# nalinbhardwaj/curdleproofs.pie

Hardware: AMD Instinct MI355X
Metric: BLS12-381 G1 scalar-muls/sec at MSM size 2^20 (higher is better)
Workload: dtype u32

## Files before the change

curdleproofs_pie_amd/csrc/capi_core_msm.h:

```cpp
#pragma once

using cg1::Ctx;
struct cg1_ctx : public cg1::Ctx {};

namespace cg1 {
static Ctx* child_of(Ctx* ctx) { return static_cast<Ctx*>(ctx->child); }

static int ensure_child(Ctx* ctx) {
  if (!ctx->child) {
    cg1_ctx* made = ctx->cu_mask.empty() ? cg1_ctx_create(ctx->device) : cg1_ctx_create_cu_mask(ctx->device, ctx->cu_mask.data(), ctx->cu_mask.size());
    if (!made) { snprintf(ctx->err, sizeof ctx->err, "could not create the second launch chain's context"); return CG1_ERR_HIP; }
    made->split = 0;
    made->batched_split = 0;
    ctx->child = made;
  }
  if (!ctx->ev_prep) HIPCHK(hipEventCreateWithFlags(&ctx->ev_prep, hipEventDisableTiming));
  if (!ctx->ev_acc) HIPCHK(hipEventCreateWithFlags(&ctx->ev_acc, hipEventDisableTiming));
  return CG1_OK;
}

static int msm_begin_split(Ctx* ctx, const PtSrc& src, const void* d_scalars32, size_t n, const WinPlan& plan, int rank, int world) {
  HIPCHK(hipSetDevice(ctx->device));
  { int crc = ensure_child(ctx); if (crc) return crc; }
  Ctx* ch = child_of(ctx);
  ch->profile = ctx->profile; ch->L0 = ctx->L0; ch->seg_m = ctx->seg_m; ch->quad = ctx->quad; ch->reduce_2d = ctx->reduce_2d;
  ch->rowcol_quad = ctx->rowcol_quad; ch->rowcol_quad_max = ctx->rowcol_quad_max; ch->fold_pass = ctx->fold_pass; ch->tree_half = ctx->tree_half; ch->tree_shift = ctx->tree_shift; ch->rowcol_lgq = ctx->rowcol_lgq; ch->tree_row = ctx->tree_row; ch->rowcol_row = ctx->rowcol_row; ch->sort_sub_bits = ctx->sort_sub_bits;
  ch->scan_one = ctx->scan_one; ch->zero_copy = ctx->zero_copy; ch->horner_threads = ctx->horner_threads; ch->host_split = ctx->host_split;
  ch->blocking_sync = ctx->blocking_sync; ch->stage_sort = ctx->stage_sort; ch->use_partition_sort = ctx->use_partition_sort; ch->big_bins = ctx->big_bins;
  const int n_own = win_count(plan.nwin, rank, world), n_lo = n_own / 2, n_hi = n_own - n_lo;
  ChainHooks hi;
  hi.after_prepare = ctx->ev_prep; hi.after_accumulate = ctx->ev_acc;
  int rc = msm_enqueue(ctx, src, d_scalars32, n, plan, rank, win_sel(world, n_lo, n_hi), hi);
  if (rc) return rc;
  PtSrc shared;
  shared.kind = PtSrc::PREPARED;
  shared.p = src.kind == PtSrc::PREPARED ? src.p : ctx->d_pts;
  shared.flags = src.kind == PtSrc::PREPARED ? src.flags : ctx->d_flags;
  ChainHooks lo;
  lo.before_start = ctx->ev_prep; lo.before_accumulate = ctx->ev_acc;
  rc = msm_enqueue(ch, shared, d_scalars32, n, plan, rank, win_sel(world, 0, n_lo), lo);
  if (rc) { snprintf(ctx->err, sizeof ctx->err, "%s", ch->err); cg1h::jac dummy; (void)msm_finish(ctx, dummy); return rc; }
  ctx->pend_split = true;
  return CG1_OK;
}
}

namespace {
struct DevBuf {
  void* p = nullptr;
  ~DevBuf() { if (p) (void)hipFree(p); }
  hipError_t alloc(size_t bytes) { return hipMalloc(&p, bytes ? bytes : 16); }
};
}

static inline cg1h::jac blob_in(const uint8_t* b) { cg1h::jac j; memcpy(&j, b, sizeof j); return j; }
static inline void blob_out(uint8_t* b, const cg1h::jac& j) { memcpy(b, &j, sizeof j); }
static_assert(sizeof(cg1h::jac) == CG1_POINT_BYTES, "point blob size");

extern "C" {

void cg1_identity(uint8_t* out) { blob_out(out, cg1h::jac_identity()); }
void cg1_generator(uint8_t* out) { blob_out(out, cg1h::jac_generator()); }
void cg1_add(uint8_t* out, const uint8_t* a, const uint8_t* b) { blob_out(out, cg1h::jac_add(blob_in(a), blob_in(b))); }
void cg1_sub(uint8_t* out, const uint8_t* a, const uint8_t* b) { blob_out(out, cg1h::jac_add(blob_in(a), cg1h::jac_neg(blob_in(b)))); }
void cg1_neg(uint8_t* out, const uint8_t* a) { blob_out(out, cg1h::jac_neg(blob_in(a))); }
void cg1_double(uint8_t* out, const uint8_t* a) { blob_out(out, cg1h::jac_dbl(blob_in(a))); }
void cg1_mul(uint8_t* out, const uint8_t* a, const uint8_t* k) { blob_out(out, cg1h::jac_mul(blob_in(a), k)); }
int cg1_eq(const uint8_t* a, const uint8_t* b) { return cg1h::jac_eq(blob_in(a), blob_in(b)) ? 1 : 0; }
int cg1_is_identity(const uint8_t* a) { return cg1h::jac_is_identity(blob_in(a)) ? 1 : 0; }
void cg1_compress(uint8_t* out48, const uint8_t* a) { cg1h::g1_compress(blob_in(a), out48); }
static int map_dec(int rc) {
  switch (rc) { case 0: return CG1_OK; case 1: case 2: return CG1_ERR_ENCODING; case 3: return CG1_ERR_NOT_ON_CURVE; default: return CG1_ERR_NOT_IN_SUBGROUP; }
}
int cg1_decompress(uint8_t* out, const uint8_t* in48, int check_subgroup) {
  cg1h::jac j;
  int rc = cg1h::g1_decompress(in48, check_subgroup != 0, j);
  if (rc == 0) blob_out(out, j);
  return map_dec(rc);
}
void cg1_to_affine96(uint8_t* out96, const uint8_t* a) {
  cg1h::fe x, y; bool inf;
  cg1h::jac_to_affine(blob_in(a), x, y, inf);
  if (inf) { memset(out96, 0, 96); return; }
  cg1h::fe_to_le48(x, out96); cg1h::fe_to_le48(y, out96 + 48);
}
int cg1_from_affine96(uint8_t* out, const uint8_t* in96, int check_on_curve) {
  bool any = false;
  for (int i = 0; i < 96; ++i) any = any || in96[i];
  if (!any) { blob_out(out, cg1h::jac_identity()); return CG1_OK; }
  cg1h::fe x, y;
  if (!cg1h::fe_from_le48(in96, x) || !cg1h::fe_from_le48(in96 + 48, y)) return CG1_ERR_ENCODING;
  cg1h::jac j = cg1h::jac_from_affine(x, y);
  if (check_on_curve && !cg1h::jac_on_curve(j)) return CG1_ERR_NOT_ON_CURVE;
  blob_out(out, j);
  return CG1_OK;
}
int cg1_batch_from_affine96(uint8_t* out_blobs, const uint8_t* in96, size_t n) {
  for (size_t i = 0; i < n; ++i) {
    int rc = cg1_from_affine96(out_blobs + CG1_POINT_BYTES * i, in96 + 96 * i, 0);
    if (rc) return rc;
  }
  return CG1_OK;
}
void cg1_batch_to_affine96(uint8_t* out96, const uint8_t* blobs, size_t n) {
  std::vector<cg1h::jac> pts(n);
  std::vector<cg1h::fe> xs(n), ys(n);
  std::vector<uint8_t> inf(n);
  for (size_t i = 0; i < n; ++i) pts[i] = blob_in(blobs + CG1_POINT_BYTES * i);
  cg1h::jac_batch_to_affine(pts.data(), n, xs.data(), ys.data(), inf.data());
  for (size_t i = 0; i < n; ++i) {
    uint8_t* o = out96 + 96 * i;
    if (inf[i]) { memset(o, 0, 96); continue; }
    cg1h::fe_to_le48(xs[i], o); cg1h::fe_to_le48(ys[i], o + 48);
  }
}
int cg1_batch_decompress(uint8_t* out_blobs, const uint8_t* in48, size_t n, int check_subgroup, size_t* bad_index) {
  for (size_t i = 0; i < n; ++i) {
    int rc = cg1_decompress(out_blobs + CG1_POINT_BYTES * i, in48 + 48 * i, check_subgroup);
    if (rc) { if (bad_index) *bad_index = i; return rc; }
  }
  return CG1_OK;
}
void cg1_batch_compress(uint8_t* out48, const uint8_t* blobs, size_t n) {
  std::vector<cg1h::jac> pts(n);
  std::vector<cg1h::fe> xs(n), ys(n);
  std::vector<uint8_t> inf(n);
  for (size_t i = 0; i < n; ++i) pts[i] = blob_in(blobs + CG1_POINT_BYTES * i);
  cg1h::jac_batch_to_affine(pts.data(), n, xs.data(), ys.data(), inf.data());
  for (size_t i = 0; i < n; ++i) {
    uint8_t* o = out48 + 48 * i;
    if (inf[i]) { memset(o, 0, 48); o[0] = 0xC0; continue; }
    cg1h::fe_to_be48(xs[i], o);
    o[0] |= 0x80;
    if (cg1h::fe_lex_largest(ys[i])) o[0] |= 0x20;
  }
}

int cg1_device_count(void) {
  int n = 0;
  if (hipGetDeviceCount(&n) != hipSuccess) return 0;
  return n;
}

cg1_ctx* cg1_ctx_create_cu_mask(int device, const uint32_t* cu_mask, size_t n_words) {
  int n = cg1_device_count();
  if (device < 0 || device >= n) return nullptr;
  if (hipSetDevice(device) != hipSuccess) return nullptr;
  cg1_ctx* ctx = new cg1_ctx();
  ctx->device = device;
  hipError_t e;
  if (cu_mask && n_words) {
    e = hipExtStreamCreateWithCUMask(&ctx->stream, (uint32_t)n_words, cu_mask);
    ctx->cu_mask.assign(cu_mask, cu_mask + n_words);
  } else {
    e = hipStreamCreateWithFlags(&ctx->stream, hipStreamNonBlocking);
  }
  if (e != hipSuccess) { delete ctx; return nullptr; }
  if (hipEventCreateWithFlags(&ctx->copy_ev, hipEventDisableTiming) != hipSuccess ||
      hipEventCreateWithFlags(&ctx->sync_ev, hipEventDisableTiming | hipEventBlockingSync) != hipSuccess) { delete ctx; return nullptr; }
  for (int i = 0; i <= CG1_NPHASE; ++i) if (hipEventCreate(&ctx->ev[i]) != hipSuccess) { delete ctx; return nullptr; }
  if (hipHostMalloc((void**)&ctx->h_flag, 64, hipHostMallocMapped | hipHostMallocCoherent) != hipSuccess || hipHostGetDevicePointer((void**)&ctx->h_flag_dev, ctx->h_flag, 0) != hipSuccess) { delete ctx; return nullptr; }
  *ctx->h_flag = 0;
  return ctx;
}
cg1_ctx* cg1_ctx_create(int device) { return cg1_ctx_create_cu_mask(device, nullptr, 0); }
void cg1_ctx_destroy(cg1_ctx* ctx) {
  if (!ctx) return;
  (void)hipSetDevice(ctx->device);
  if (ctx->child) { cg1_ctx_destroy(ctx->child); ctx->child = nullptr; }
  if (ctx->ev_prep) (void)hipEventDestroy(ctx->ev_prep);
  if (ctx->ev_acc) (void)hipEventDestroy(ctx->ev_acc);
  cg1::free_bufs(ctx);
  if (ctx->d_merlin_rows) (void)hipFree(ctx->d_merlin_rows);
  if (ctx->d_opening) (void)hipFree(ctx->d_opening);
  if (ctx->d_prover) (void)hipFree(ctx->d_prover);
  if (ctx->d_gen_tab) (void)hipFree(ctx->d_gen_tab);
  if (ctx->d_small_partial) (void)hipFree(ctx->d_small_partial);
  if (ctx->d_small_ctr) (void)hipFree(ctx->d_small_ctr);
  if (ctx->d_small_pts) (void)hipFree(ctx->d_small_pts);
  if (ctx->d_small_flags) (void)hipFree(ctx->d_small_flags);
  if (ctx->h_small_out) (void)hipHostFree(ctx->h_small_out);
  if (ctx->d_stage_pts) (void)hipFree(ctx->d_stage_pts);
  if (ctx->d_stage_sc) (void)hipFree(ctx->d_stage_sc);
  if (ctx->h_flag) (void)hipHostFree(ctx->h_flag);
  for (int i = 0; i <= CG1_NPHASE; ++i) (void)hipEventDestroy(ctx->ev[i]);
  (void)hipStreamDestroy(ctx->stream);
  if (ctx->copy_ev) (void)hipEventDestroy(ctx->copy_ev);
  if (ctx->sync_ev) (void)hipEventDestroy(ctx->sync_ev);
  for (int i = 0; i < 2; ++i) if (ctx->tm_ev[i]) (void)hipEventDestroy(ctx->tm_ev[i]);
  if (ctx->copy_stream.load()) (void)hipStreamDestroy(ctx->copy_stream.load());
  if (ctx->side_ev) (void)hipEventDestroy(ctx->side_ev);
  if (ctx->side_stream) (void)hipStreamDestroy(ctx->side_stream);
  delete ctx;
}
const char* cg1_ctx_error(const cg1_ctx* ctx) { return ctx ? ctx->err : "null context (no GPU visible?)"; }

void* cg1_dev_malloc(cg1_ctx* ctx, size_t bytes) {
  if (!ctx) return nullptr;
  void* p = nullptr;
  if (hipSetDevice(ctx->device) != hipSuccess || hipMalloc(&p, bytes ? bytes : 16) != hipSuccess) return nullptr;
  return p;
}
void cg1_dev_free(cg1_ctx* ctx, void* p) { if (ctx && p) { (void)hipSetDevice(ctx->device); (void)hipFree(p); } }
int cg1_h2d(cg1_ctx* ctx, void* dst, const void* src, size_t bytes) {
  if (!ctx) return CG1_ERR_HIP;
  HIPCHK(hipSetDevice(ctx->device));
  HIPCHK(hipMemcpy(dst, src, bytes, hipMemcpyHostToDevice));
  return CG1_OK;
}
int cg1_d2h(cg1_ctx* ctx, void* dst, const void* src, size_t bytes) {
  if (!ctx) return CG1_ERR_HIP;
  HIPCHK(hipSetDevice(ctx->device));
  HIPCHK(hipMemcpy(dst, src, bytes, hipMemcpyDeviceToHost));
  return CG1_OK;
}
int cg1_h2d_async(cg1_ctx* ctx, void* dst, const void* src, size_t bytes) {
  if (!ctx) return CG1_ERR_HIP;
  if (bytes == 0) return CG1_OK;
  HIPCHK(hipSetDevice(ctx->device));
  std::call_once(ctx->copy_once, [ctx]() { hipStream_t s = nullptr; if (hipStreamCreateWithFlags(&s, hipStreamNonBlocking) == hipSuccess) ctx->copy_stream.store(s); });
  hipStream_t cs = ctx->copy_stream.load();
  if (!cs) { snprintf(ctx->err, sizeof ctx->err, "could not create the copy stream"); return CG1_ERR_HIP; }
  HIPCHK(hipMemcpyAsync(dst, src, bytes, hipMemcpyHostToDevice, cs));
  return CG1_OK;
}
int cg1_stream_sync(cg1_ctx* ctx) {
  if (!ctx) return CG1_ERR_HIP;
  HIPCHK(hipSetDevice(ctx->device));
  return cg1::wait_stream(ctx);
}
int cg1_copy_fence(cg1_ctx* ctx) {
  if (!ctx) return CG1_ERR_HIP;
  HIPCHK(hipSetDevice(ctx->device));
  hipStream_t cs = ctx->copy_stream.load();
  if (!cs) return CG1_OK;
  HIPCHK(hipEventRecord(ctx->copy_ev, cs));
  HIPCHK(hipStreamWaitEvent(ctx->stream, ctx->copy_ev, 0));
  return CG1_OK;
}
void* cg1_host_alloc(cg1_ctx* ctx, size_t bytes) {
  if (!ctx) return nullptr;
  void* p = nullptr;
  if (hipSetDevice(ctx->device) != hipSuccess) return nullptr;
  if (hipHostMalloc(&p, bytes ? bytes : 1) != hipSuccess) return nullptr;
  return p;
}
void cg1_host_free(cg1_ctx* ctx, void* p) {
  if (!ctx || !p) return;
  (void)hipSetDevice(ctx->device);
  (void)hipHostFree(p);
}
int cg1_d2h_2d(cg1_ctx* ctx, void* dst, size_t dst_pitch, const void* src, size_t src_pitch, size_t width, size_t rows) {
  if (!ctx) return CG1_ERR_HIP;
  if (rows == 0 || width == 0) return CG1_OK;
  if (width > dst_pitch || width > src_pitch) return CG1_ERR_ARG;
  HIPCHK(hipSetDevice(ctx->device));
  HIPCHK(hipMemcpy2D(dst, dst_pitch, src, src_pitch, width, rows, hipMemcpyDeviceToHost));
  return CG1_OK;
}
int cg1_ctx_sync(cg1_ctx* ctx) {
  if (!ctx) return CG1_ERR_HIP;
  HIPCHK(hipSetDevice(ctx->device));
  HIPCHK(hipDeviceSynchronize());
  return CG1_OK;
}
int cg1_merlin_last_passes(const cg1_ctx* ctx) { return ctx ? (int)ctx->merlin_passes : -1; }
int cg1_merlin_last_kernel(const cg1_ctx* ctx) { return ctx ? ctx->merlin_last_kernel : -1; }
int cg1_ctx_device(const cg1_ctx* ctx) { return ctx ? ctx->device : -1; }
void* cg1_ctx_stream(cg1_ctx* ctx) { return ctx ? (void*)ctx->stream : nullptr; }
int cg1_ctx_set_param(cg1_ctx* ctx, const char* name, int value) {
  if (!ctx || !name) return CG1_ERR_ARG;
  if (!strcmp(name, "chunk_rule")) { ctx->chunk_rule = value != 0; return CG1_OK; }
  if (!strcmp(name, "chunk_len")) { if (value < 1 || value > 65536) return CG1_ERR_ARG; ctx->L0 = (uint32_t)value; cg1::free_bufs(ctx); return CG1_OK; }
  if (!strcmp(name, "stage_sort")) { ctx->stage_sort = value ? 1 : 0; return CG1_OK; }
  if (!strcmp(name, "quad")) { ctx->quad = value ? 1 : 0; return CG1_OK; }
  if (!strcmp(name, "glv")) { if (value < 0 || value > 2) return CG1_ERR_ARG; ctx->glv = value; return CG1_OK; }
  if (!strcmp(name, "glv_max_n")) { if (value < 0) return CG1_ERR_ARG; ctx->glv_max_n = value; return CG1_OK; }
  if (!strcmp(name, "batched_split")) { ctx->batched_split = value ? 1 : 0; return CG1_OK; }
  if (!strcmp(name, "batched_split_min_m")) { if (value < 2) return CG1_ERR_ARG; ctx->batched_split_min_m = value; return CG1_OK; }
  if (!strcmp(name, "lincomb_zero_copy")) { ctx->lincomb_zero_copy = value ? 1 : 0; return CG1_OK; }
  if (!strcmp(name, "fold_quad")) { ctx->fold_quad = value ? 1 : 0; return CG1_OK; }
  if (!strcmp(name, "rowcol_row")) { ctx->rowcol_row = value ? 1 : 0; return CG1_OK; }
  if (!strcmp(name, "tree_row")) { ctx->tree_row = value ? 1 : 0; return CG1_OK; }
  if (!strcmp(name, "horner_row")) { ctx->horner_row = value ? 1 : 0; return CG1_OK; }
  if (!strcmp(name, "batch_mul_row")) { ctx->batch_mul_row = value ? 1 : 0; return CG1_OK; }
  if (!strcmp(name, "small_msm")) { ctx->small_msm = value ? 1 : 0; return CG1_OK; }
  if (!strcmp(name, "fixed_slice")) { if (value < 0 || value > 128) return CG1_ERR_ARG; ctx->fixed_slice = value; return CG1_OK; }
  if (!strcmp(name, "fixed_waves")) { if (value != 0 && value != 4 && value != 8 && value != 16) return CG1_ERR_ARG; ctx->fixed_waves = value; return CG1_OK; }
  if (!strcmp(name, "ipa_inv")) { if (value != 0 && value != 1) return CG1_ERR_ARG; ctx->ipa_inv = value; return CG1_OK; }
  if (!strcmp(name, "small_row_tail")) { ctx->small_row_tail = value ? 1 : 0; return CG1_OK; }
  if (!strcmp(name, "split")) { ctx->split = value ? 1 : 0; return CG1_OK; }
  if (!strcmp(name, "split_min_log2n")) { if (value < 10 || value > 31) return CG1_ERR_ARG; ctx->split_min_n = (size_t)1 << value; return CG1_OK; }
  if (!strcmp(name, "reduce_2d")) { ctx->reduce_2d = value ? 1 : 0; return CG1_OK; }
  if (!strcmp(name, "partition_sort")) { ctx->use_partition_sort = value ? 1 : 0; cg1::free_bufs(ctx); return CG1_OK; }
  if (!strcmp(name, "blocking_sync")) { ctx->blocking_sync = value != 0; return CG1_OK; }
  if (!strcmp(name, "big_bins")) { ctx->big_bins = value != 0; return CG1_OK; }
  if (!strcmp(name, "host_split")) { ctx->host_split = value != 0; return CG1_OK; }
  if (!strcmp(name, "arm_helpers")) { ctx->arm_helpers = value != 0; return CG1_OK; }
  if (!strcmp(name, "horner_threads")) { if (value != 1 && value != 2 && value != 4) return CG1_ERR_ARG; ctx->horner_threads = value; return CG1_OK; }
  if (!strcmp(name, "zero_copy")) { ctx->zero_copy = value != 0; return CG1_OK; }
  if (!strcmp(name, "auto_plan")) { ctx->auto_plan = value != 0; return CG1_OK; }
  if (!strcmp(name, "rowcol_quad")) { ctx->rowcol_quad = value != 0; return CG1_OK; }
  if (!strcmp(name, "rowcol_quad_max")) { if (value < 0) return CG1_ERR_ARG; ctx->rowcol_quad_max = value; return CG1_OK; }
  if (!strcmp(name, "fold_pass")) { ctx->fold_pass = value != 0; return CG1_OK; }
  if (!strcmp(name, "scan_one")) { ctx->scan_one = value != 0; return CG1_OK; }
  if (!strcmp(name, "batched_host_horner_max")) { if (value < 0) return CG1_ERR_ARG; ctx->batched_host_horner_max = value; return CG1_OK; }
  if (!strcmp(name, "tree_shift")) { if (value < -1 || value > 4) return CG1_ERR_ARG; ctx->tree_shift = value; return CG1_OK; }
  if (!strcmp(name, "rowcol_lgq")) { if (value != 0 && (value < 2 || value > 4)) return CG1_ERR_ARG; ctx->rowcol_lgq = value; return CG1_OK; }
  if (!strcmp(name, "sort_sub_bits")) { if (value != 0 && (value < 4 || value > 8)) return CG1_ERR_ARG; ctx->sort_sub_bits = value; return CG1_OK; }
  if (!strcmp(name, "batch_mul_host_max")) { if (value < -1) return CG1_ERR_ARG; ctx->batch_mul_host_max = value; return CG1_OK; }
  if (!strcmp(name, "batch_mul_quad_max")) { if (value < 0) return CG1_ERR_ARG; ctx->batch_mul_quad_max = value; return CG1_OK; }
  if (!strcmp(name, "merlin_sync")) { ctx->merlin_sync = value != 0; return CG1_OK; }
  if (!strcmp(name, "fe_timed")) { ctx->fe_timed = value != 0; return CG1_OK; }
  if (!strcmp(name, "fe_rows")) { ctx->fe_rows = value != 0; return CG1_OK; }
  if (!strcmp(name, "fe_prio")) { if (value < 0 || value > 3) return CG1_ERR_ARG; ctx->fe_prio = value; return CG1_OK; }
  if (!strcmp(name, "decompress_waves")) { if (value != 2 && value != 3) return CG1_ERR_ARG; ctx->decompress_waves = value; return CG1_OK; }
  if (!strcmp(name, "merlin_rows")) { ctx->merlin_rows = value != 0; return CG1_OK; }
  if (!strcmp(name, "merlin_lanes")) { if (value < 1 || value > 64) return CG1_ERR_ARG; ctx->merlin_lanes = value; return CG1_OK; }
  if (!strcmp(name, "tree_half")) { ctx->tree_half = value != 0; return CG1_OK; }
  if (!strcmp(name, "wave_agg")) {
    int v = value ? 1 : 0;
    HIPCHK(hipSetDevice(ctx->device));
    HIPCHK(hipMemcpyToSymbol(HIP_SYMBOL(cg1::g_wave_agg), &v, sizeof v));
    return CG1_OK;
  }
  if (!strcmp(name, "profile")) { if (value < 0 || value > 2) return CG1_ERR_ARG; ctx->profile = value; return CG1_OK; }
  if (!strcmp(name, "seg_m")) { if (value != 1 && value != 2 && value != 4 && value != 8 && value != 16) return CG1_ERR_ARG; ctx->seg_m = (uint32_t)value; return CG1_OK; }
  return CG1_ERR_ARG;
}

int cg1_msm_device(cg1_ctx* ctx, const void* d_points, const void* d_scalars, size_t n, int window_c, int shard_rank,
                   int shard_world, uint8_t* out) {
  if (!ctx) return CG1_ERR_HIP;
  cg1h::jac r;
  int rc = cg1::msm_device(ctx, d_points, d_scalars, n, window_c, shard_rank, shard_world, r);
  if (rc == CG1_OK) blob_out(out, r);
  return rc;
}

int cg1_msm_device_begin(cg1_ctx* ctx, const void* d_points, const void* d_scalars, size_t n, int window_c, int shard_rank, int shard_world) {
  if (!ctx) return CG1_ERR_HIP;
  return cg1::msm_begin(ctx, d_points, d_scalars, n, window_c, shard_rank, shard_world);
}
int cg1_msm_device_end(cg1_ctx* ctx, uint8_t* out) {
  if (!ctx) return CG1_ERR_HIP;
  cg1h::jac r;
  int rc = cg1::msm_end(ctx, r);
  if (rc == CG1_OK) blob_out(out, r);
  return rc;
}

int cg1_msm_multi_device(cg1_ctx* const* ctxs, size_t n_ctx, const void* const* d_points, const void* const* d_scalars, const size_t* n,
                         int window_c, uint8_t* out) {
  if (!ctxs || !n_ctx || !d_points || !d_scalars || !n || !out) return CG1_ERR_ARG;
  for (size_t i = 0; i < n_ctx; ++i) {
    if (!ctxs[i]) return CG1_ERR_HIP;
    for (size_t j = 0; j < i; ++j) if (ctxs[j] == ctxs[i]) return CG1_ERR_ARG;
  }
  int rc = CG1_OK;
  size_t begun = 0;
  for (; begun < n_ctx && rc == CG1_OK; ++begun)
    rc = cg1::msm_begin(ctxs[begun], d_points[begun], d_scalars[begun], n[begun], window_c, 0, 1);
  cg1h::jac acc = cg1h::jac_identity();
  for (size_t i = 0; i < begun; ++i) {
    cg1h::jac part;
    int r2 = cg1::msm_end(ctxs[i], part);
    if (rc == CG1_OK) rc = r2;
    if (r2 == CG1_OK) acc = cg1h::jac_add(acc, part);
  }
  if (rc == CG1_OK) blob_out(out, acc);
  return rc;
}

static int ensure_stage(cg1_ctx* ctx, size_t pts_bytes, size_t sc_bytes) {
  if (pts_bytes > ctx->cap_stage_pts) {
    if (ctx->d_stage_pts) (void)hipFree(ctx->d_stage_pts);
    ctx->d_stage_pts = nullptr; ctx->cap_stage_pts = 0;
    const size_t want = pts_bytes + pts_bytes / 4 + 256;
    HIPCHK(hipMalloc(&ctx->d_stage_pts, want));
    ctx->cap_stage_pts = want;
  }
  if (sc_bytes > ctx->cap_stage_sc) {
    if (ctx->d_stage_sc) (void)hipFree(ctx->d_stage_sc);
    ctx->d_stage_sc = nullptr; ctx->cap_stage_sc = 0;
    const size_t want = sc_bytes + sc_bytes / 4 + 256;
    HIPCHK(hipMalloc(&ctx->d_stage_sc, want));
    ctx->cap_stage_sc = want;
  }
  return CG1_OK;
}

static int ensure_lin(cg1_ctx* ctx, size_t bytes) {
  if (bytes <= ctx->cap_h_lin) return CG1_OK;
  if (ctx->h_lin) (void)hipHostFree(ctx->h_lin);
  ctx->h_lin = nullptr; ctx->h_lin_dev = nullptr; ctx->cap_h_lin = 0;
  const size_t want = bytes + bytes / 4 + 4096;
  HIPCHK(hipHostMalloc((void**)&ctx->h_lin, want, hipHostMallocMapped));
  HIPCHK(hipHostGetDevicePointer((void**)&ctx->h_lin_dev, ctx->h_lin, 0));
  ctx->cap_h_lin = want;
  return CG1_OK;
}

int cg1_msm(cg1_ctx* ctx, const uint8_t* points, const uint8_t* scalars, size_t n, uint8_t* out) {
  if (!ctx) return CG1_ERR_HIP;
  if (n == 0) { blob_out(out, cg1h::jac_identity()); return CG1_OK; }
  HIPCHK(hipSetDevice(ctx->device));
  if (n <= 4096 && ctx->lincomb_zero_copy) {
    { int lrc = ensure_lin(ctx, n * 128); if (lrc) return lrc; }
    memcpy(ctx->h_lin, points, n * 96);
    memcpy(ctx->h_lin + n * 96, scalars, n * 32);
    return cg1_msm_device(ctx, ctx->h_lin_dev, ctx->h_lin_dev + n * 96, n, 0, 0, 1, out);
  }
  { int src = ensure_stage(ctx, n * 96, n * 32); if (src) return src; }
  HIPCHK(hipMemcpyAsync(ctx->d_stage_pts, points, n * 96, hipMemcpyHostToDevice, ctx->stream));
  HIPCHK(hipMemcpyAsync(ctx->d_stage_sc, scalars, n * 32, hipMemcpyHostToDevice, ctx->stream));
  return cg1_msm_device(ctx, ctx->d_stage_pts, ctx->d_stage_sc, n, 0, 0, 1, out);
}

int cg1_msm_blobs(cg1_ctx* ctx, const uint8_t* blobs144, const uint8_t* scalars32, size_t n, int all_normalised, uint8_t* out) {
  if (!ctx) return CG1_ERR_HIP;
  if (n == 0) { blob_out(out, cg1h::jac_identity()); return CG1_OK; }
  if (!blobs144 || !scalars32) return CG1_ERR_ARG;
  HIPCHK(hipSetDevice(ctx->device));
  { int src = ensure_stage(ctx, n * CG1_POINT_BYTES, n * 32); if (src) return src; }
  HIPCHK(hipMemcpyAsync(ctx->d_stage_pts, blobs144, n * CG1_POINT_BYTES, hipMemcpyHostToDevice, ctx->stream));
  HIPCHK(hipMemcpyAsync(ctx->d_stage_sc, scalars32, n * 32, hipMemcpyHostToDevice, ctx->stream));
  cg1::PtSrc src;
  src.kind = cg1::PtSrc::BLOBS; src.p = ctx->d_stage_pts; src.normalised = all_normalised != 0;
  cg1h::jac r;
  int rc = cg1::msm_device(ctx, src, ctx->d_stage_sc, n, 0, 0, 1, r);
  if (rc == CG1_OK) blob_out(out, r);
  return rc;
}
int cg1_stage_reserve(cg1_ctx* ctx, size_t pts_bytes, size_t sc_bytes, void** d_pts, void** d_sc) {
  if (!ctx) return CG1_ERR_HIP;
  HIPCHK(hipSetDevice(ctx->device));
  { int src = ensure_stage(ctx, pts_bytes, sc_bytes); if (src) return src; }
  if (d_pts) *d_pts = ctx->d_stage_pts;
  if (d_sc) *d_sc = ctx->d_stage_sc;
  return CG1_OK;
}
int cg1_msm_blobs_device(cg1_ctx* ctx, const void* d_blobs144, const void* d_scalars32, size_t n, int all_normalised, uint8_t* out) {
  if (!ctx) return CG1_ERR_HIP;
  if (n == 0) { blob_out(out, cg1h::jac_identity()); return CG1_OK; }
  if (!d_blobs144 || !d_scalars32) return CG1_ERR_ARG;
  HIPCHK(hipSetDevice(ctx->device));
  cg1::PtSrc src;
  src.kind = cg1::PtSrc::BLOBS; src.p = d_blobs144; src.normalised = all_normalised != 0;
  cg1h::jac r;
  int rc = cg1::msm_device(ctx, src, d_scalars32, n, 0, 0, 1, r);
  if (rc == CG1_OK) blob_out(out, r);
  return rc;
}
}
```

curdleproofs_pie_amd/csrc/host_chains.h:

```cpp
#pragma once

namespace cg1 {

static WinPlan make_plan(int c, bool glv = false) {
  WinPlan pl;
  const int bits = glv ? 127 : 255;
  pl.glv = glv ? 1 : 0;
  if (c > 0) { pl.cmax = c; pl.nwin = bits / c + 1; pl.n_hi = pl.nwin; }
  else {
    const int cm = -c, nw = (bits + 1 + cm - 1) / cm;
    pl.cmax = cm; pl.nwin = nw; pl.n_hi = bits + 1 - nw * (cm - 1);
    if (pl.n_hi < 0) pl.n_hi = 0;
  }
  return pl;
}

static int pick_plan_c(size_t n, int auto_plan) {
  const int c = pick_window(n);
  if (!auto_plan || c != 16) return c;
  if (n <= (1u << 14)) return -12;
  if (n <= (3u << 15)) return -13;
  if (n <= (3u << 16)) return -15;
  return 16;
}

int pick_window(size_t n) {
  if (n <= 128) return 4;
  if (n <= 8192) return 8;
  return 16;
}

static int wait_stream(Ctx* ctx) {
  if (ctx->blocking_sync) {
    HIPCHK(hipEventRecord(ctx->sync_ev, ctx->stream));
    HIPCHK(hipEventSynchronize(ctx->sync_ev));
    return CG1_OK;
  }
  HIPCHK(hipStreamSynchronize(ctx->stream));
  return CG1_OK;
}

struct PtSrc {
  enum Kind { AFFINE96 = 0, BLOBS = 1, PREPARED = 2 } kind = AFFINE96;
  const void* p = nullptr;
  const uint8_t* flags = nullptr;
  bool normalised = false;
  PtSrc() {}
  PtSrc(const void* affine96) : p(affine96) {}
};

static uint32_t blob_points_per_lane(size_t n) {
  size_t K = (n + (1u << 17) - 1) >> 17;
  return (uint32_t)(K < 1 ? 1 : (K > 16 ? 16 : K));
}

static void launch_prepare(hipStream_t st, const PtSrc& src, PreparedPoint* out, uint8_t* flags_out, uint32_t n32, uint32_t* status_words) {
  if (src.kind == PtSrc::AFFINE96) {
    hipLaunchKernelGGL(k_prepare_points, dim3((n32 + 255) / 256), dim3(256), 0, st, (const uint32_t*)src.p, out, flags_out, n32, status_words);
  } else if (src.normalised) {
    hipLaunchKernelGGL((k_prepare_blobs<false>), dim3((n32 + 127) / 128), dim3(128), 0, st, (const uint32_t*)src.p, out, flags_out, n32, 1u, status_words);
  } else {
    const uint32_t K = blob_points_per_lane(n32);
    const uint32_t lanes = (n32 + K - 1) / K;
    hipLaunchKernelGGL((k_prepare_blobs<true>), dim3((lanes + 127) / 128), dim3(128), 0, st, (const uint32_t*)src.p, out, flags_out, n32, K, status_words);
  }
}

struct ChainHooks {
  hipEvent_t before_start = nullptr, after_prepare = nullptr, before_accumulate = nullptr, after_accumulate = nullptr;
};

static int msm_enqueue(Ctx* ctx, const PtSrc& src, const void* d_scalars32, size_t n, const WinPlan& plan, int rank, int world,
                       const ChainHooks& hooks = ChainHooks()) {
  ctx->pend.active = false;
  HIPCHK(hipSetDevice(ctx->device));
  const int c = plan.cmax, nwin = plan.nwin;
  const size_t n_real = n;
  if (plan.glv) n *= 2;
  const int nlw = win_count(nwin, rank, world);
  if (nlw <= 0) return CG1_OK;
  const uint32_t NB = 1u << (c - 1);
  const uint32_t m = std::min<uint32_t>(ctx->seg_m, NB);
  const uint32_t J = NB / m;
  int nbits = 0; while ((1u << nbits) < J) ++nbits;
  const uint32_t bb = (uint32_t)c - 1u, lb2 = (bb + 1u) / 2u, hb2 = bb - lb2;
  const bool use2d = ctx->reduce_2d != 0;
  const uint32_t nitems = use2d ? 1u + hb2 + lb2 : 1u + (uint32_t)nbits;
  const size_t nb_total = (size_t)nlw * NB;
  uint32_t L0 = ctx->L0;
  while (L0 < 65536u && ((uint64_t)n * (uint64_t)nlw >> 18) > (uint64_t)L0) L0 <<= 1;
  if (ctx->chunk_rule && world == 1) {
    const uint64_t entries = (uint64_t)n * (uint64_t)nlw;
    if (entries >= (1ull << 20) && entries < (1ull << 21) && L0 < 10u) L0 = 10u;
    if (entries >= (1ull << 21) && entries < (1ull << 24) && nb_total > (size_t)ctx->rowcol_quad_max) {
      const double mload = (double)n / (double)(1u << bb);
      uint32_t want = (uint32_t)(mload + 8.0 * std::sqrt(mload) + 1.0);
      if (entries < (1ull << 22) && want > 20u) want = 20u;
      if (want > L0) L0 = want;
    }
  }
  int rc = ensure(ctx, n, nb_total, nlw, nitems, L0, src.kind != PtSrc::PREPARED);
  if (rc) return rc;
  hipStream_t st = ctx->stream;
  const uint32_t n32 = (uint32_t)n;
  const uint32_t gn = (n32 + 255) / 256;
  const int profile = ctx->profile;
  auto h0 = std::chrono::steady_clock::now();
  const bool resident = src.kind == PtSrc::PREPARED;
  const PreparedPoint* pts = resident ? static_cast<const PreparedPoint*>(src.p) : ctx->d_pts;
  const uint8_t* flags = resident ? src.flags : ctx->d_flags;
  const size_t nout_words = (size_t)nlw * nitems;
  uint32_t* bad_flag = reinterpret_cast<uint32_t*>(ctx->d_out + nout_words);
  if (hooks.before_start) HIPCHK(hipStreamWaitEvent(st, hooks.before_start, 0));
  if (profile >= 2) HIPCHK(hipEventRecord(ctx->ev[0], st));
  const uint32_t n_real32 = (uint32_t)n_real;
  if (resident) HIPCHK(hipMemsetAsync(bad_flag, 0, 16, st));
  else {
    launch_prepare(st, src, ctx->d_pts, ctx->d_flags, n_real32, bad_flag);
    if (plan.glv) hipLaunchKernelGGL(k_phi_records, dim3((n_real32 + 255) / 256), dim3(256), 0, st, ctx->d_pts, ctx->d_flags, n_real32);
  }
  if (hooks.after_prepare) HIPCHK(hipEventRecord(hooks.after_prepare, st));
  if (profile >= 2) HIPCHK(hipEventRecord(ctx->ev[1], st));
  const uint32_t nblk = (uint32_t)((nb_total + SCAN_ITEMS - 1) / SCAN_ITEMS);
  if (ctx->use_partition_sort && n <= PART_MAX_N) {
    const uint32_t want_sub = ctx->sort_sub_bits ? (uint32_t)ctx->sort_sub_bits : (n <= ((size_t)1 << 16) ? 7u : 8u);
    uint32_t sub_bits = bb < want_sub ? bb : want_sub;
    while (bb - sub_bits > 7u) ++sub_bits;
    const uint32_t nbins = 1u << (bb - sub_bits);
    const uint32_t nslices = (n32 + PART_TILE - 1) / PART_TILE;
    const uint32_t nbc = (uint32_t)nlw * nbins * nslices;
    hipLaunchKernelGGL(k_digits, dim3((n_real32 + 255) / 256), dim3(256), 0, st, (const uint32_t*)d_scalars32, flags, ctx->d_digits, n_real32, plan, rank, world, bad_flag);
    hipLaunchKernelGGL(k_part_count, dim3(nslices, nlw), dim3(256), 0, st, ctx->d_digits, ctx->d_blockcnt, n32, nslices, nbins, sub_bits);
    const uint32_t ublk = (nbc + SCAN_ITEMS - 1) / SCAN_ITEMS;
    if (ctx->scan_one && nbc <= USCAN1_MAX) {
      hipLaunchKernelGGL(k_uscan_one, dim3(1), dim3(1024), 0, st, ctx->d_blockcnt, nbc);
    } else {
      hipLaunchKernelGGL(k_uscan1, dim3(ublk), dim3(256), 0, st, ctx->d_blockcnt, ctx->d_ublocktot, nbc);
      hipLaunchKernelGGL(k_uscan2, dim3(1), dim3(256), 0, st, ctx->d_ublocktot, ublk, ctx->d_blockcnt, nbc);
      hipLaunchKernelGGL(k_uscan3, dim3(ublk), dim3(256), 0, st, ctx->d_ublocktot, ctx->d_blockcnt, nbc);
    }
    if (profile >= 2) HIPCHK(hipEventRecord(ctx->ev[2], st));
    hipLaunchKernelGGL(k_part_scatter, dim3(nslices, nlw), dim3(256), 0, st, ctx->d_digits, ctx->d_blockcnt, ctx->d_part, n32, nslices, nbins, sub_bits, ctx->stage_sort);
    const uint32_t nbt = (uint32_t)nlw * nbins;
    const int big_bins = ctx->big_bins && n32 > 2u * BIN_STAGE;
    hipLaunchKernelGGL(k_slice_plan, dim3(1), dim3(256), 0, st, ctx->d_blockcnt, nbt, nslices, ctx->d_slice_base, ctx->d_bigflag, big_bins);
    hipLaunchKernelGGL(k_bin_sort, dim3(nbt), dim3(256), 0, st, ctx->d_part, ctx->d_blockcnt, ctx->d_hist, ctx->d_sorted, nbt, nslices, sub_bits, ctx->stage_sort, ctx->d_bigflag);
    if (big_bins) {
      const uint32_t max_slices = (uint32_t)(((size_t)n * (size_t)nlw) / SLICE + nbt + 1);
      hipLaunchKernelGGL(k_slice_count, dim3(max_slices), dim3(256), 0, st, ctx->d_part, ctx->d_blockcnt, nbt, nslices, ctx->d_slice_base, ctx->d_slicehist);
      hipLaunchKernelGGL(k_slice_prefix, dim3(nbt), dim3(256), 0, st, ctx->d_blockcnt, nslices, sub_bits, ctx->d_slice_base, ctx->d_bigflag, ctx->d_slicehist, ctx->d_subbase, ctx->d_hist);
      hipLaunchKernelGGL(k_slice_scatter, dim3(max_slices), dim3(256), 0, st, ctx->d_part, ctx->d_blockcnt, nbt, nslices, ctx->d_slice_base, ctx->d_slicehist, ctx->d_subbase, ctx->d_sorted);
    }
    if (profile >= 2) HIPCHK(hipEventRecord(ctx->ev[3], st));
    if (ctx->scan_one && nb_total <= SCAN1_MAX) {
      hipLaunchKernelGGL(k_scan_one, dim3(1), dim3(1024), 0, st, ctx->d_hist, ctx->d_off, ctx->d_choff, (uint32_t)nb_total, L0);
    } else {
      hipLaunchKernelGGL(k_scan1, dim3(nblk), dim3(256), 0, st, ctx->d_hist, ctx->d_off, ctx->d_choff, ctx->d_blocktot, (uint32_t)nb_total, L0);
      hipLaunchKernelGGL(k_scan2, dim3(1), dim3(256), 0, st, ctx->d_blocktot, nblk, ctx->d_off, ctx->d_choff, (uint32_t)nb_total);
      hipLaunchKernelGGL(k_scan3, dim3(nblk), dim3(256), 0, st, ctx->d_blocktot, ctx->d_off, ctx->d_choff, (uint32_t)nb_total);
    }
  } else {
    HIPCHK(hipMemsetAsync(ctx->d_hist, 0, nb_total * 4, st));
    hipLaunchKernelGGL(k_hist, dim3(gn), dim3(256), 0, st, (const uint32_t*)d_scalars32, flags, ctx->d_hist, n32, plan, rank, world, bad_flag);
    if (profile >= 2) HIPCHK(hipEventRecord(ctx->ev[2], st));
    hipLaunchKernelGGL(k_scan1, dim3(nblk), dim3(256), 0, st, ctx->d_hist, ctx->d_off, ctx->d_choff, ctx->d_blocktot, (uint32_t)nb_total, L0);
    hipLaunchKernelGGL(k_scan2, dim3(1), dim3(256), 0, st, ctx->d_blocktot, nblk, ctx->d_off, ctx->d_choff, (uint32_t)nb_total);
    hipLaunchKernelGGL(k_scan3, dim3(nblk), dim3(256), 0, st, ctx->d_blocktot, ctx->d_off, ctx->d_choff, (uint32_t)nb_total);
    if (profile >= 2) HIPCHK(hipEventRecord(ctx->ev[3], st));
    hipLaunchKernelGGL(k_scatter, dim3(gn), dim3(256), 0, st, (const uint32_t*)d_scalars32, flags, ctx->d_hist, ctx->d_off, ctx->d_sorted, n32, plan, rank, world);
  }
  HIPCHK(hipMemsetAsync(ctx->d_zblock, 0, zblock_clear_bytes(ctx), st));
  hipLaunchKernelGGL(k_chunk_desc, dim3((uint32_t)std::min<size_t>(CHUNK_DESC_BLOCKS, (nb_total + 255) / 256)), dim3(256), 0, st, ctx->d_off, ctx->d_choff, ctx->d_desc, ctx->d_lenhist, ctx->d_heavy, (uint32_t)ctx->cap_heavy, (uint32_t)nb_total, L0, ctx->d_any_multi);
  const size_t max_chunks = nb_total + (n * (size_t)nlw) / L0 + 1;
  const uint32_t gchunks = (uint32_t)((max_chunks + 255) / 256);
  hipLaunchKernelGGL(k_len_scan, dim3(1), dim3(256), 0, st, ctx->d_lenhist, ctx->d_lenhist + LEN_BINS, ctx->d_off + nb_total, ctx->d_choff + nb_total, bad_flag);
  hipLaunchKernelGGL(k_order, dim3((gchunks + ORDER_PER - 1) / ORDER_PER), dim3(256), 0, st, ctx->d_desc, ctx->d_choff + nb_total, ctx->d_lenhist + LEN_BINS, ctx->d_order);
  if (hooks.before_accumulate) HIPCHK(hipStreamWaitEvent(st, hooks.before_accumulate, 0));
  if (profile >= 1) HIPCHK(hipEventRecord(ctx->ev[4], st));
  hipLaunchKernelGGL(k_accumulate, dim3(gchunks), dim3(256), 0, st, ctx->d_desc, ctx->d_choff + nb_total, ctx->d_order, ctx->d_sorted, pts, ctx->d_sums);
  if (profile >= 1) HIPCHK(hipEventRecord(ctx->ev[5], st));
  if (hooks.after_accumulate) HIPCHK(hipEventRecord(hooks.after_accumulate, st));
  hipLaunchKernelGGL(k_heavy_combine, dim3(512), dim3(256), 0, st, ctx->d_heavy, (uint32_t)ctx->cap_heavy, ctx->d_choff, ctx->d_sums, ctx->d_combined);
  const bool small_quad = ctx->quad && ctx->rowcol_quad && nb_total <= (size_t)ctx->rowcol_quad_max;
  const bool rows_fold = small_quad && use2d && ctx->rowcol_row && ctx->tree_row && nb_total <= 8192;
  if (rows_fold) {}
  else if (small_quad && ctx->fold_quad)
    hipLaunchKernelGGL(k_bucket_fold_quad, dim3((uint32_t)((nb_total * 4 + 255) / 256)), dim3(256), 0, st, ctx->d_choff, ctx->d_sums, ctx->d_combined, (uint32_t)nb_total, ctx->d_any_multi);
  else if (ctx->fold_pass)
    hipLaunchKernelGGL(k_bucket_fold, dim3((uint32_t)((nb_total + 255) / 256)), dim3(256), 0, st, ctx->d_choff, ctx->d_sums, ctx->d_combined, (uint32_t)nb_total, ctx->d_any_multi);
  bool tree_exports = false;
  if (use2d) {
    const uint32_t R = 1u << hb2, Cn = 1u << lb2;
    const uint32_t lpr = Cn < 32u ? Cn : 32u, lpc = R < 16u ? R : 16u;
    const uint32_t nrow_blocks = ((uint32_t)nlw * R + (256u / lpr) - 1u) / (256u / lpr);
    const uint32_t ncol_blocks = ((uint32_t)nlw * Cn + (256u / lpc) - 1u) / (256u / lpc);
    PointSum* rowsum = ctx->d_segrun;
    PointSum* colsum = ctx->d_segtot;
    if (small_quad) {
      uint32_t lgq = (R == Cn) ? 2u : 3u;
      if (ctx->rowcol_lgq >= 2 && ctx->rowcol_lgq <= 4) lgq = (uint32_t)ctx->rowcol_lgq;
      const uint32_t rc_waves = ((uint32_t)nlw * (R + Cn) + (16u >> lgq) - 1u) / (16u >> lgq);
      if (ctx->rowcol_row && ctx->tree_row)
        hipLaunchKernelGGL(k_rowcol_quad_row, dim3(((uint32_t)nlw * (R + Cn) + 3u) / 4u), dim3(256), 0, st, ctx->d_choff, ctx->d_sums, ctx->d_combined,
                           rowsum, colsum, (uint32_t)nlw, hb2, lb2);
      else
      hipLaunchKernelGGL(k_rowcol_quad, dim3((rc_waves + 3u) / 4u), dim3(256), 0, st, ctx->d_choff, ctx->d_sums,
                         rowsum, colsum, (uint32_t)nlw, hb2, lb2, lgq);
    }
    else
      hipLaunchKernelGGL(k_rowcol, dim3(nrow_blocks + ncol_blocks), dim3(256), 0, st, ctx->d_choff, ctx->d_sums, ctx->d_combined,
                         rowsum, colsum, (uint32_t)nlw, hb2, lb2, nrow_blocks, ctx->quad);
    if (profile >= 2) HIPCHK(hipEventRecord(ctx->ev[6], st));
    const uint32_t tree_threads = std::min<uint32_t>(512u, std::max<uint32_t>(64u, 4u << std::max(hb2, lb2)) >> (ctx->tree_shift >= 0 ? ctx->tree_shift : (ctx->tree_half ? 1 : 0)));
    if (ctx->tree_row) {
      uint32_t W = (1u << std::max(hb2, lb2)) >> 3;
      W = W < 1u ? 1u : (W > 16u ? 16u : W);
      tree_exports = ctx->zero_copy != 0;
      if (tree_exports) ++ctx->seq;
      hipLaunchKernelGGL(k_small_tree_row, dim3(nitems, nlw), dim3(64u * W), 0, st, rowsum, colsum, ctx->d_out, hb2, lb2,
                         tree_exports ? ctx->h_out_dev : (PointWords*)nullptr, bad_flag, ctx->h_flag_dev, ctx->seq);
    }
    else if (ctx->quad) hipLaunchKernelGGL(k_small_tree_quad, dim3(nitems, nlw), dim3(std::max<uint32_t>(64u, tree_threads)), 0, st, rowsum, colsum, ctx->d_out, hb2, lb2);
    else hipLaunchKernelGGL(k_small_tree, dim3(nitems, nlw), dim3(256), 0, st, rowsum, colsum, ctx->d_out, hb2, lb2);
  } else {
    const uint32_t nseg_total = (uint32_t)(nb_total / m);
    hipLaunchKernelGGL(k_seg_reduce, dim3((nseg_total + 255) / 256), dim3(256), 0, st, ctx->d_choff, ctx->d_sums, ctx->d_combined, ctx->d_segrun, ctx->d_segtot, nseg_total, m);
    if (profile >= 2) HIPCHK(hipEventRecord(ctx->ev[6], st));
    uint32_t S = (J + BT_ELEMS - 1) / BT_ELEMS; if (S < 1) S = 1; if (S > 64) S = 64;
    hipLaunchKernelGGL(k_bit_tree, dim3(nitems, nlw, S), dim3(256), 0, st, ctx->d_segrun, ctx->d_segtot, ctx->d_partial, J);
    hipLaunchKernelGGL(k_bit_tree_final, dim3((uint32_t)(nitems * nlw)), dim3(64), 0, st, ctx->d_partial, ctx->d_out, S);
  }
  const bool zc = ctx->zero_copy != 0;
  if (zc && tree_exports) {
  } else if (zc) {
    ++ctx->seq;
    const uint32_t nvec = (uint32_t)((((size_t)nlw * nitems + 1) * sizeof(PointWords)) / 16);
    hipLaunchKernelGGL(k_export_host, dim3(1), dim3(1024), 0, st, reinterpret_cast<const uint4*>(ctx->d_out), reinterpret_cast<uint4*>(ctx->h_out_dev), nvec,
                       ctx->h_flag_dev, ctx->seq);
  } else {
    HIPCHK(hipMemcpyAsync(ctx->h_out, ctx->d_out, ((size_t)nlw * nitems + 1) * sizeof(PointWords), hipMemcpyDeviceToHost, st));
  }
  if (profile >= 2) HIPCHK(hipEventRecord(ctx->ev[7], st));
  auto h1 = std::chrono::steady_clock::now();
  Ctx::Pending& pd = ctx->pend;
  pd.zero_copy = zc; pd.seq = ctx->seq; pd.hout = ctx->h_out;
  pd.active = true; pd.c = c; pd.plan = plan; pd.rank = rank; pd.world = world; pd.nlw = nlw; pd.nbits = nbits; pd.m = m; pd.lb2 = lb2; pd.hb2 = hb2;
  pd.nitems = nitems; pd.use2d = use2d; pd.profile = profile; pd.nout_words = nout_words; pd.h0 = h0; pd.h1 = h1;
  pd.arm_helpers = ctx->arm_helpers && ctx->host_split && ctx->horner_threads > 1 && n <= ((size_t)1 << 18);
  return CG1_OK;
}

static int msm_finish(Ctx* ctx, cg1h::jac& result) {
  result = cg1h::jac_identity();
  if (!ctx->pend.active) return CG1_OK;
  const Ctx::Pending pd = ctx->pend;
  ctx->pend.active = false;
  const int c = pd.c, rank = pd.rank, world = pd.world, nlw = pd.nlw, nbits = pd.nbits;
  (void)c;
  const uint32_t m = pd.m, lb2 = pd.lb2, hb2 = pd.hb2, nitems = pd.nitems;
  const bool use2d = pd.use2d;
  const size_t nout_words = pd.nout_words;
  const auto h0 = pd.h0, h1 = pd.h1;
  HIPCHK(hipSetDevice(ctx->device));
  struct StandDown { Ctx* c; bool on; ~StandDown() { if (on) for (int j = 0; j < 3; ++j) c->helper[j].disarm(); } } stand_down{ctx, false};
  if (pd.zero_copy && !ctx->blocking_sync && pd.profile < 2) {
    if (pd.arm_helpers) for (int j = 0; j < 3 && j + 1 < ctx->horner_threads; ++j) ctx->helper[j].arm();
    stand_down.on = pd.arm_helpers;
    volatile uint32_t* flag = ctx->h_flag;
    for (uint32_t spins = 0; *flag != pd.seq; ++spins) {
      if ((spins & 0x3fffu) == 0x3fffu) {
        hipError_t q = hipStreamQuery(ctx->stream);
        if (q == hipSuccess) { if (*flag != pd.seq) { snprintf(ctx->err, sizeof ctx->err, "the stream drained without the export flag"); return CG1_ERR_HIP; } break; }
        if (q != hipErrorNotReady) { snprintf(ctx->err, sizeof ctx->err, "stream failed: %s", hipGetErrorString(q)); return CG1_ERR_HIP; }
      }
      __builtin_ia32_pause();
    }
    std::atomic_thread_fence(std::memory_order_acquire);
  } else {
    int wrc = wait_stream(ctx); if (wrc) return wrc;
  }
  HIPCHK(hipGetLastError());
  {
    const uint32_t* st_words = reinterpret_cast<const uint32_t*>(pd.hout + nout_words);
    ctx->last_entries = st_words[1]; ctx->last_chunks = st_words[2];
    if (st_words[0]) {
      snprintf(ctx->err, sizeof ctx->err, "a scalar is >= 2^255: scalar32 must be a canonical Fr element (< r)");
      return CG1_ERR_ENCODING;
    }
  }
  auto h2 = std::chrono::steady_clock::now();
  { int erc = read_phase_events(ctx, pd.profile); if (erc) return erc; }
  ctx->last_c = c;

  auto t0 = std::chrono::steady_clock::now();
  ctx->host_ms[0] = std::chrono::duration<float, std::milli>(h1 - h0).count();
  ctx->host_ms[1] = std::chrono::duration<float, std::milli>(h2 - h1).count();
  ctx->host_ms[2] = std::chrono::duration<float, std::milli>(t0 - h2).count();
  int lm = 0; while ((1u << lm) < m) ++lm;
  const WinPlan& plan = pd.plan;
  constexpr int EMAX = 2 * 256 + 64;
  std::vector<std::pair<int, const PointWords*>> items;
  items.reserve((size_t)nlw * nitems);
  int e_top = 0;
  for (int lw = 0; lw < nlw; ++lw) {
    const int w = win_global(lw, rank, world), base = plan.off(w);
    const PointWords* row = pd.hout + (size_t)lw * nitems;
    auto put = [&](int e, const PointWords* p) { if (!p->inf && e >= 0 && e < EMAX) { items.emplace_back(e, p); if (e > e_top) e_top = e; } };
    put(base, &row[0]);
    if (use2d) {
      for (uint32_t k = 0; k < hb2; ++k) put(base + (int)lb2 + (int)k, &row[1 + k]);
      for (uint32_t k = 0; k < lb2; ++k) put(base + (int)k, &row[1 + hb2 + k]);
    } else {
      for (int b2 = 0; b2 < nbits; ++b2) put(base + lm + b2, &row[1 + b2]);
    }
  }
  uint16_t first[EMAX + 1];
  memset(first, 0, sizeof first);
  for (const auto& it : items) ++first[it.first + 1];
  for (int e = 0; e < EMAX; ++e) first[e + 1] = (uint16_t)(first[e + 1] + first[e]);
  std::vector<const PointWords*> byexp(items.size());
  {
    uint16_t cur[EMAX];
    memcpy(cur, first, sizeof cur);
    for (const auto& it : items) byexp[cur[it.first]++] = it.second;
  }
  auto horner = [&](int lo, int hi) {
    cg1h::jac a = cg1h::jac_identity();
    for (int e = hi; e >= lo; --e) {
      a = cg1h::jac_dbl(a);
      for (uint16_t k = first[e]; k < first[e + 1]; ++k) a = cg1h::jac_add(a, jac_from_words(*byexp[k]));
    }
    return a;
  };
  cg1h::jac acc;
  const int nth = (!ctx->host_split || e_top < 96) ? 1 : (ctx->horner_threads >= 4 && e_top >= 112 ? 4 : 2);
  if (nth > 1) {
    cg1h::jac part[4];
    int lo[5];
    {
      constexpr long DBL = 7, ADD = 16;
      auto fill = [&](long C, int* cut) {
        int e = 0;
        for (int j = 0; j < nth; ++j) {
          cut[j] = e;
          long adds = 0;
          while (e <= e_top && DBL * (e + 1) + ADD * (adds + (first[e + 1] - first[e])) <= C) { adds += first[e + 1] - first[e]; ++e; }
        }
        cut[nth] = e_top + 1;
        return e > e_top;
      };
      long lo_c = DBL * (e_top + 1), hi_c = DBL * (e_top + 1) + ADD * (long)items.size();
      int cut[5];
      while (lo_c < hi_c) {
        const long mid = (lo_c + hi_c) / 2;
        if (fill(mid, cut)) hi_c = mid; else lo_c = mid + 1;
      }
      fill(hi_c, cut);
      for (int j = 0; j <= nth; ++j) lo[j] = cut[j];
    }
    auto run_part = [&](int j) {
      cg1h::jac a = horner(lo[j], lo[j + 1] - 1);
      for (int k = 0; k < lo[j]; ++k) a = cg1h::jac_dbl(a);
      part[j] = a;
    };
    for (int j = 0; j + 1 < nth; ++j) ctx->helper[j].run([&, j]() { run_part(j); });
    if (pd.arm_helpers) for (int j = nth - 1 < 0 ? 0 : nth - 1; j < 3; ++j) ctx->helper[j].disarm();
    run_part(nth - 1);
    acc = part[nth - 1];
    for (int j = 0; j + 1 < nth; ++j) { ctx->helper[j].wait(); acc = cg1h::jac_add(acc, part[j]); }
  } else {
    if (pd.arm_helpers) for (int j = 0; j < 3; ++j) ctx->helper[j].disarm();
    acc = horner(0, e_top);
  }
  result = acc;
  ctx->host_tail_ms = std::chrono::duration<float, std::milli>(std::chrono::steady_clock::now() - t0).count();
  ctx->host_ms[3] = ctx->host_tail_ms;
  return CG1_OK;
}

static int pick_small_c(size_t n) {
  if (n <= 24) return 4;
  if (n <= 96) return 6;
  if (n <= 6 * SM_SLICE) return 7;
  return 8;
}

static int msm_enqueue_small(Ctx* ctx, const PtSrc& src, const void* d_scalars32, size_t n, int c, uint32_t M = 1, const uint32_t* d_offs = nullptr, size_t max_n = 0,
                             bool glv = false) {
  ctx->pend.active = false;
  HIPCHK(hipSetDevice(ctx->device));
  const WinPlan plan = make_plan(c, glv);
  const uint32_t nwin = (uint32_t)plan.nwin, bb = (uint32_t)c - 1u, lb2 = (bb + 1u) / 2u, hb2 = bb - lb2, nitems = 1u + hb2 + lb2;
  if (M == 1) max_n = n;
  const uint32_t S = (uint32_t)(((glv ? 2 * max_n : max_n) + SM_SLICE - 1) / SM_SLICE);
  auto h0 = std::chrono::steady_clock::now();
  if (!ctx->h_small_out) {
    HIPCHK(hipHostMalloc((void**)&ctx->h_small_out, ((size_t)SM_MAX_MSMS * 64 * 9 + 1) * sizeof(PointWords), hipHostMallocMapped | hipHostMallocCoherent));
    HIPCHK(hipHostGetDevicePointer((void**)&ctx->h_small_out_dev, ctx->h_small_out, 0));
    HIPCHK(hipMalloc(&ctx->d_small_ctr, (SM_MAX_MSMS * 64 + 8) * 4));
    HIPCHK(hipMemsetAsync(ctx->d_small_ctr, 0, (SM_MAX_MSMS * 64 + 8) * 4, ctx->stream));
  }
  const size_t need_partial = (size_t)M * nwin * S * nitems;
  if (S > 1 && need_partial > ctx->cap_small_partial) {
    if (ctx->d_small_partial) (void)hipFree(ctx->d_small_partial);
    ctx->d_small_partial = nullptr; ctx->cap_small_partial = 0;
    HIPCHK(hipMalloc(&ctx->d_small_partial, need_partial * sizeof(PointSum)));
    ctx->cap_small_partial = need_partial;
  }
  hipStream_t st = ctx->stream;
  SmallArgs a;
  a.src = src.p; a.flags = src.flags; a.scalars = static_cast<const uint32_t*>(d_scalars32); a.offs = d_offs;
  a.n = (uint32_t)n; a.M = M; a.S = S; a.c = (uint32_t)c; a.nwin = nwin; a.hb = hb2; a.lb = lb2; a.nitems = nitems;
  a.partial = ctx->d_small_partial; a.counters = ctx->d_small_ctr;
  a.out_host = ctx->h_small_out_dev; a.flag_host = ctx->h_flag_dev; a.seq = ++ctx->seq;
  a.row_tail = ctx->small_row_tail ? 1u : 0u;
  a.glv = glv ? 1u : 0u;
  int kind = (int)src.kind;
  if (src.kind == PtSrc::BLOBS && !src.normalised) {
    if (n > ctx->cap_small_pts) {
      if (ctx->d_small_pts) (void)hipFree(ctx->d_small_pts);
      if (ctx->d_small_flags) (void)hipFree(ctx->d_small_flags);
      ctx->d_small_pts = nullptr; ctx->d_small_flags = nullptr; ctx->cap_small_pts = 0;
      const size_t cap = n < SM_MAX_N ? SM_MAX_N : n;
      HIPCHK(hipMalloc(&ctx->d_small_pts, cap * sizeof(PreparedPoint)));
      HIPCHK(hipMalloc(&ctx->d_small_flags, cap + 16));
      ctx->cap_small_pts = cap;
    }
    launch_prepare(st, src, ctx->d_small_pts, ctx->d_small_flags, (uint32_t)n, nullptr);
    a.src = ctx->d_small_pts; a.flags = ctx->d_small_flags;
    kind = (int)PtSrc::PREPARED;
  }
  const dim3 grid(nwin, S, M), block(512);
  if (kind == (int)PtSrc::AFFINE96) hipLaunchKernelGGL((k_msm_small<0>), grid, block, 0, st, a);
  else if (kind == (int)PtSrc::BLOBS) hipLaunchKernelGGL((k_msm_small<1>), grid, block, 0, st, a);
  else hipLaunchKernelGGL((k_msm_small<2>), grid, block, 0, st, a);
  auto h1 = std::chrono::steady_clock::now();
  Ctx::Pending& pd = ctx->pend;
  pd.zero_copy = true; pd.seq = ctx->seq; pd.hout = ctx->h_small_out;
  pd.active = true; pd.c = c; pd.plan = plan; pd.rank = 0; pd.world = 1; pd.nlw = (int)nwin; pd.nbits = 0; pd.m = 1; pd.lb2 = lb2; pd.hb2 = hb2;
  pd.nitems = nitems; pd.use2d = true; pd.profile = 0; pd.nout_words = (size_t)M * nwin * nitems; pd.h0 = h0; pd.h1 = h1;
  pd.arm_helpers = ctx->arm_helpers && ctx->host_split && ctx->horner_threads > 1 && M == 1;
  return CG1_OK;
}

static cg1h::jac horner_2d_items(const PointWords* rows, const WinPlan& plan, uint32_t nitems, uint32_t hb2, uint32_t lb2) {
  constexpr int EMAX = 2 * 256 + 64;
  std::vector<std::pair<int, const PointWords*>> items;
  items.reserve((size_t)plan.nwin * nitems);
  int e_top = 0;
  for (int w = 0; w < plan.nwin; ++w) {
    const int base = plan.off(w);
    const PointWords* row = rows + (size_t)w * nitems;
    auto put = [&](int e, const PointWords* p) { if (!p->inf) { items.emplace_back(e, p); if (e > e_top) e_top = e; } };
    put(base, &row[0]);
    for (uint32_t k = 0; k < hb2; ++k) put(base + (int)lb2 + (int)k, &row[1 + k]);
    for (uint32_t k = 0; k < lb2; ++k) put(base + (int)k, &row[1 + hb2 + k]);
  }
  uint16_t first[EMAX + 1];
  memset(first, 0, sizeof first);
  for (const auto& it : items) ++first[it.first + 1];
  for (int e = 0; e < EMAX; ++e) first[e + 1] = (uint16_t)(first[e + 1] + first[e]);
  std::vector<const PointWords*> byexp(items.size());
  {
    uint16_t cur[EMAX];
    memcpy(cur, first, sizeof cur);
    for (const auto& it : items) byexp[cur[it.first]++] = it.second;
  }
  cg1h::jac a = cg1h::jac_identity();
  for (int e = e_top; e >= 0; --e) {
    a = cg1h::jac_dbl(a);
    for (uint16_t k = first[e]; k < first[e + 1]; ++k) a = cg1h::jac_add(a, jac_from_words(*byexp[k]));
  }
  return a;
}

static int msm_small_batched_finish(Ctx* ctx, uint32_t M, std::vector<cg1h::jac>& results) {
  const Ctx::Pending pd = ctx->pend;
  ctx->pend.active = false;
  HIPCHK(hipSetDevice(ctx->device));
  if (!ctx->blocking_sync) {
    volatile uint32_t* flag = ctx->h_flag;
    for (uint32_t spins = 0; *flag != pd.seq; ++spins) {
      if ((spins & 0x3fffu) == 0x3fffu) {
        hipError_t q = hipStreamQuery(ctx->stream);
        if (q == hipSuccess) { if (*flag != pd.seq) { snprintf(ctx->err, sizeof ctx->err, "the stream drained without the export flag"); return CG1_ERR_HIP; } break; }
        if (q != hipErrorNotReady) { snprintf(ctx->err, sizeof ctx->err, "stream failed: %s", hipGetErrorString(q)); return CG1_ERR_HIP; }
      }
      __builtin_ia32_pause();
    }
    std::atomic_thread_fence(std::memory_order_acquire);
  } else {
    int wrc = wait_stream(ctx); if (wrc) return wrc;
  }
  HIPCHK(hipGetLastError());
  const uint32_t* st_words = reinterpret_cast<const uint32_t*>(pd.hout + pd.nout_words);
  ctx->last_entries = st_words[1]; ctx->last_chunks = 0;
  if (st_words[0]) {
    snprintf(ctx->err, sizeof ctx->err, "a scalar is >= 2^255: scalar32 must be a canonical Fr element (< r)");
    return CG1_ERR_ENCODING;
  }
  auto t0 = std::chrono::steady_clock::now();
  const size_t per = (size_t)pd.plan.nwin * pd.nitems;
  auto one = [&](size_t j) { results[j] = horner_2d_items(pd.hout + j * per, pd.plan, pd.nitems, pd.hb2, pd.lb2); };
  if (M <= 4) {
    const size_t nth = std::min<size_t>(4, M);
    for (size_t t = 1; t < nth; ++t) ctx->helper[t - 1].run([&, t]() { for (size_t j = t; j < M; j += nth) one(j); });
    for (size_t j = 0; j < M; j += nth) one(j);
    for (size_t t = 1; t < nth; ++t) ctx->helper[t - 1].wait();
  } else {
    std::atomic<size_t> next{0};
    std::function<void()> work = [&]() { for (;;) { const size_t j = next.fetch_add(1); if (j >= M) return; one(j); } };
    Pool& pool = Pool::get();
    pool.run(work, std::min<size_t>(M, pool.size() + 1));
  }
  auto t1 = std::chrono::steady_clock::now();
  ctx->host_ms[0] = std::chrono::duration<float, std::milli>(pd.h1 - pd.h0).count();
  ctx->host_ms[1] = std::chrono::duration<float, std::milli>(t0 - pd.h1).count();
  ctx->host_ms[2] = 0;
  ctx->host_ms[3] = ctx->host_tail_ms = std::chrono::duration<float, std::milli>(t1 - t0).count();
  for (int i = 0; i < CG1_NPHASE; ++i) ctx->phase_ms[i] = 0.f;
  ctx->last_c = pd.c;
  ctx->last_acc_launches = 0;
  return CG1_OK;
}

static Ctx* child_of(Ctx* ctx);
static int msm_begin_split(Ctx* ctx, const PtSrc& src, const void* d_scalars32, size_t n, const WinPlan& plan, int rank, int world);

int msm_begin(Ctx* ctx, const PtSrc& src, const void* d_scalars32, size_t n, int c, int rank, int world) {
  ctx->pend.active = false;
  ctx->pend_c = 0;
  if (n == 0) return CG1_OK;
  if (n >= (1ull << 31)) { snprintf(ctx->err, sizeof ctx->err, "n too large"); return CG1_ERR_ARG; }
  if (world < 1 || world > 255 || rank < 0 || rank >= world) { snprintf(ctx->err, sizeof ctx->err, "bad window shard %d/%d", rank, world); return CG1_ERR_ARG; }
  for (int pass = (ctx->glv && 2 * n <= SM_MAX_N) ? 1 : 0; pass >= 0; --pass) {
    const bool sglv = pass == 1;
    const size_t nn = sglv ? 2 * n : n;
    const int bits = sglv ? 127 : 255;
    if (ctx->small_msm && nn <= SM_MAX_N && world == 1 && (c == 0 || (c >= 4 && c <= 9 && c != 5)) &&
        (size_t)(bits / (c ? c : pick_small_c(nn)) + 1) * ((nn + SM_SLICE - 1) / SM_SLICE) <= SM_ONE_ROUND) {
      if (c == 0) c = pick_small_c(nn);
      ctx->pend_c = c;
      return msm_enqueue_small(ctx, src, d_scalars32, n, c, 1, nullptr, 0, sglv);
    }
  }
  const bool glv = src.kind != PtSrc::PREPARED && ctx->use_partition_sort && 2 * n <= PART_MAX_N &&
                   (ctx->glv == 2 || (ctx->glv == 1 && n <= (size_t)ctx->glv_max_n));
  if (c == 0) c = pick_plan_c(glv ? 2 * n : n, ctx->auto_plan);
  const int cabs = c < 0 ? -c : c;
  if (cabs < 4 || cabs > 16) { snprintf(ctx->err, sizeof ctx->err, "window width %d out of range [4,16]", c); return CG1_ERR_ARG; }
  const WinPlan plan = make_plan(c, glv);
  ctx->pend_c = c;
  ctx->pend_split = false;
  if (ctx->split && n >= ctx->split_min_n && win_count(plan.nwin, rank, world) >= 2) return msm_begin_split(ctx, src, d_scalars32, n, plan, rank, world);
  return msm_enqueue(ctx, src, d_scalars32, n, plan, rank, world);
}
int msm_end(Ctx* ctx, cg1h::jac& result) {
  const bool was_small = ctx->pend.active && ctx->pend.hout == ctx->h_small_out;
  int rc = msm_finish(ctx, result);
  ctx->last_acc_launches = ctx->pend_split ? 2 : (was_small ? 0 : 1);
  if (ctx->pend_split) {
    ctx->pend_split = false;
    Ctx* ch = child_of(ctx);
    const float acc_hi = ctx->phase_ms[4], wait_hi = ctx->host_ms[1], tail_hi = ctx->host_ms[3], enq = ctx->host_ms[0];
    const uint32_t e_hi = ctx->last_entries, c_hi = ctx->last_chunks;
    cg1h::jac lo;
    int rc2 = msm_finish(ch, lo);
    if (rc == CG1_OK) rc = rc2;
    if (rc2 != CG1_OK) snprintf(ctx->err, sizeof ctx->err, "%s", ch->err);
    if (rc == CG1_OK) result = cg1h::jac_add(result, lo);
    for (int i = 0; i < CG1_NPHASE; ++i) ctx->phase_ms[i] += ch->phase_ms[i];
    ctx->phase_ms[4] = acc_hi + ch->phase_ms[4];
    ctx->last_entries = e_hi + ch->last_entries; ctx->last_chunks = c_hi + ch->last_chunks;
    ctx->host_ms[0] = enq + ch->host_ms[0]; ctx->host_ms[1] = wait_hi + ch->host_ms[1]; ctx->host_ms[3] = tail_hi + ch->host_ms[3];
    ctx->host_tail_ms = ch->host_ms[3];
  }
  if (ctx->pend_c) ctx->last_c = ctx->pend_c;
  return rc;
}
int msm_device(Ctx* ctx, const PtSrc& src, const void* d_scalars32, size_t n, int c, int rank, int world, cg1h::jac& result) {
  result = cg1h::jac_identity();
  int rc = msm_begin(ctx, src, d_scalars32, n, c, rank, world);
  if (rc) return rc;
  return msm_end(ctx, result);
}


int pick_window_batched(size_t n_avg, bool glv) {
  const int bits = glv ? 127 : 255;
  if (glv) n_avg *= 2;
  int best = 4; double best_cost = 1e300;
  for (int c = 4; c <= 9; ++c) {
    if (bits % c == 0) continue;
    int nwin = bits / c + 1;
    double NB = (double)(1u << (c - 1));
    double cost = (double)nwin * ((double)n_avg + 1.4 * (2.0 * NB + 3.0 * NB / 8.0)) + 1.4 * (double)bits;
    if (cost < best_cost) { best_cost = cost; best = c; }
  }
  return best;
}
int pick_window_batched(size_t n_avg) { return pick_window_batched(n_avg, false); }

static int ensure_child(Ctx* ctx);

struct BatchedChain {
  size_t M = 0; int c = 0; uint32_t nwin = 0; bool host_horner = false;
  std::chrono::steady_clock::time_point h0, h1;
};
static int batched_chain_enqueue(Ctx* ctx, const void* d_points96, const void* d_scalars32, const uint32_t* h_offsets, size_t M, int c, bool glv,
                                 hipEvent_t wait_before_accumulate, hipEvent_t record_after_accumulate, BatchedChain& bc) {
  const size_t N = h_offsets[M], N_real = N;
  HIPCHK(hipSetDevice(ctx->device));
  const WinPlan bplan = make_plan(c, glv);
  const uint32_t nwin = (uint32_t)bplan.nwin, NB = 1u << (c - 1);
  const size_t G = M * nwin, nb_total = G * NB;
  const size_t Nv = glv ? 2 * N : N;
  if (nb_total >= (1ull << 31) || Nv * nwin >= (1ull << 31)) { snprintf(ctx->err, sizeof ctx->err, "batch too large"); return CG1_ERR_ARG; }
  const uint32_t m = 8 < NB ? 8 : NB;
  uint32_t log2m = 0; while ((1u << log2m) < m) ++log2m;
  const uint32_t J = NB / m;
  uint32_t L0 = ctx->L0;
  while (L0 < 65536u && ((uint64_t)Nv * (uint64_t)nwin >> 18) > (uint64_t)L0) L0 <<= 1;
  int rc = ensure(ctx, Nv, nb_total, nwin, 1, L0);
  if (rc) return rc;
  if ((M + 1) > ctx->cap_boffs) {
    if (ctx->d_boffs) (void)hipFree(ctx->d_boffs);
    HIPCHK(hipMalloc(&ctx->d_boffs, (M + 1) * 4));
    ctx->cap_boffs = M + 1;
  }
  if (G > ctx->cap_gsum) {
    if (ctx->d_gsum) (void)hipFree(ctx->d_gsum);
    HIPCHK(hipMalloc(&ctx->d_gsum, G * sizeof(PointSum)));
    ctx->cap_gsum = G;
  }
  if (M > ctx->cap_bout) {
    if (ctx->d_bout) (void)hipFree(ctx->d_bout);
    if (ctx->h_bout) (void)hipHostFree(ctx->h_bout);
    HIPCHK(hipMalloc(&ctx->d_bout, (M + 1) * sizeof(PointWords)));
    HIPCHK(hipHostMalloc(&ctx->h_bout, (M + 1) * sizeof(PointWords)));
    ctx->cap_bout = M;
  }
  if (Nv * nwin > ctx->cap_digits) {
    if (ctx->d_digits) (void)hipFree(ctx->d_digits);
    HIPCHK(hipMalloc(&ctx->d_digits, Nv * nwin * 2 + 16));
    ctx->cap_digits = Nv * nwin;
  }
  hipStream_t st = ctx->stream;
  const uint32_t N32 = (uint32_t)N_real, gn = (N32 + 255) / 256, Nv32 = (uint32_t)Nv, split = glv ? N32 : 0u;
  auto h0 = std::chrono::steady_clock::now();
  HIPCHK(hipMemcpyAsync(ctx->d_boffs, h_offsets, (M + 1) * 4, hipMemcpyHostToDevice, st));
  if (ctx->profile >= 2) HIPCHK(hipEventRecord(ctx->ev[0], st));
  uint32_t* bad_flag = reinterpret_cast<uint32_t*>(ctx->d_bout + M);
  hipLaunchKernelGGL(k_prepare_points, dim3(gn), dim3(256), 0, st, (const uint32_t*)d_points96, ctx->d_pts, ctx->d_flags, N32, bad_flag);
  if (glv) hipLaunchKernelGGL(k_phi_records, dim3(gn), dim3(256), 0, st, ctx->d_pts, ctx->d_flags, N32);
  if (ctx->profile >= 2) HIPCHK(hipEventRecord(ctx->ev[1], st));
  hipLaunchKernelGGL(k_digits, dim3(gn), dim3(256), 0, st, (const uint32_t*)d_scalars32, ctx->d_flags, ctx->d_digits, N32, bplan, 0, 1, bad_flag);
  hipLaunchKernelGGL(k_group_count, dim3((uint32_t)M, nwin), dim3(256), 0, st, ctx->d_digits, ctx->d_boffs, ctx->d_hist, Nv32, NB, nwin, split);
  if (ctx->profile >= 2) HIPCHK(hipEventRecord(ctx->ev[2], st));
  const uint32_t nblk = (uint32_t)((nb_total + SCAN_ITEMS - 1) / SCAN_ITEMS);
  hipLaunchKernelGGL(k_scan1, dim3(nblk), dim3(256), 0, st, ctx->d_hist, ctx->d_off, ctx->d_choff, ctx->d_blocktot, (uint32_t)nb_total, L0);
  hipLaunchKernelGGL(k_scan2, dim3(1), dim3(256), 0, st, ctx->d_blocktot, nblk, ctx->d_off, ctx->d_choff, (uint32_t)nb_total);
  hipLaunchKernelGGL(k_scan3, dim3(nblk), dim3(256), 0, st, ctx->d_blocktot, ctx->d_off, ctx->d_choff, (uint32_t)nb_total);
  hipLaunchKernelGGL(k_group_scatter, dim3((uint32_t)M, nwin), dim3(256), 0, st, ctx->d_digits, ctx->d_boffs, ctx->d_off, ctx->d_sorted, Nv32, NB, nwin, split);
  if (ctx->profile >= 2) HIPCHK(hipEventRecord(ctx->ev[3], st));
  HIPCHK(hipMemsetAsync(ctx->d_zblock, 0, zblock_clear_bytes(ctx), st));
  hipLaunchKernelGGL(k_chunk_desc, dim3((uint32_t)std::min<size_t>(CHUNK_DESC_BLOCKS, (nb_total + 255) / 256)), dim3(256), 0, st, ctx->d_off, ctx->d_choff, ctx->d_desc, ctx->d_lenhist, ctx->d_heavy, (uint32_t)ctx->cap_heavy, (uint32_t)nb_total, L0, ctx->d_any_multi);
  const size_t max_chunks = nb_total + (Nv * (size_t)nwin) / L0 + 1;
  const uint32_t gchunks = (uint32_t)((max_chunks + 255) / 256);
  hipLaunchKernelGGL(k_len_scan, dim3(1), dim3(256), 0, st, ctx->d_lenhist, ctx->d_lenhist + LEN_BINS, ctx->d_off + nb_total, ctx->d_choff + nb_total, bad_flag);
  hipLaunchKernelGGL(k_order, dim3((gchunks + ORDER_PER - 1) / ORDER_PER), dim3(256), 0, st, ctx->d_desc, ctx->d_choff + nb_total, ctx->d_lenhist + LEN_BINS, ctx->d_order);
  if (wait_before_accumulate) HIPCHK(hipStreamWaitEvent(st, wait_before_accumulate, 0));
  if (ctx->profile >= 1) HIPCHK(hipEventRecord(ctx->ev[4], st));
  hipLaunchKernelGGL(k_accumulate, dim3(gchunks), dim3(256), 0, st, ctx->d_desc, ctx->d_choff + nb_total, ctx->d_order, ctx->d_sorted, ctx->d_pts, ctx->d_sums);
  if (ctx->profile >= 1) HIPCHK(hipEventRecord(ctx->ev[5], st));
  if (record_after_accumulate) HIPCHK(hipEventRecord(record_after_accumulate, st));
  const uint32_t nseg_total = (uint32_t)(nb_total / m);
  hipLaunchKernelGGL(k_heavy_combine, dim3(512), dim3(256), 0, st, ctx->d_heavy, (uint32_t)ctx->cap_heavy, ctx->d_choff, ctx->d_sums, ctx->d_combined);
  hipLaunchKernelGGL(k_seg_reduce, dim3((nseg_total + 255) / 256), dim3(256), 0, st, ctx->d_choff, ctx->d_sums, ctx->d_combined, ctx->d_segrun, ctx->d_segtot, nseg_total, m);
  hipLaunchKernelGGL(k_group_reduce, dim3((uint32_t)((G + 255) / 256)), dim3(256), 0, st, ctx->d_segrun, ctx->d_segtot, ctx->d_gsum, (uint32_t)G, J, log2m);
  if (ctx->profile >= 2) HIPCHK(hipEventRecord(ctx->ev[6], st));
  const bool host_horner = M <= (size_t)ctx->batched_host_horner_max;
  if (host_horner) {
    if (G > ctx->cap_gout) {
      if (ctx->d_gout) (void)hipFree(ctx->d_gout);
      if (ctx->h_gout) (void)hipHostFree(ctx->h_gout);
      ctx->d_gout = nullptr; ctx->h_gout = nullptr; ctx->cap_gout = 0;
      HIPCHK(hipMalloc(&ctx->d_gout, G * sizeof(PointWords)));
      HIPCHK(hipHostMalloc(&ctx->h_gout, G * sizeof(PointWords)));
      ctx->cap_gout = G;
    }
    hipLaunchKernelGGL(k_export_sums, dim3((uint32_t)((G + 63) / 64)), dim3(64), 0, st, ctx->d_gsum, ctx->d_gout, (uint32_t)G);
    HIPCHK(hipMemcpyAsync(ctx->h_gout, ctx->d_gout, G * sizeof(PointWords), hipMemcpyDeviceToHost, st));
    HIPCHK(hipMemcpyAsync(ctx->h_bout + M, ctx->d_bout + M, sizeof(PointWords), hipMemcpyDeviceToHost, st));
  } else {
    if (ctx->horner_row && M <= 2048) hipLaunchKernelGGL(k_msm_horner_row, dim3((uint32_t)M), dim3(64), 0, st, ctx->d_gsum, ctx->d_bout, (uint32_t)M, nwin, (uint32_t)c);
    else if (ctx->quad) hipLaunchKernelGGL(k_msm_horner_quad, dim3((uint32_t)((M * 4 + 63) / 64)), dim3(64), 0, st, ctx->d_gsum, ctx->d_bout, (uint32_t)M, nwin, (uint32_t)c);
    else hipLaunchKernelGGL(k_msm_horner, dim3((uint32_t)((M + 63) / 64)), dim3(64), 0, st, ctx->d_gsum, ctx->d_bout, (uint32_t)M, nwin, (uint32_t)c);
    HIPCHK(hipMemcpyAsync(ctx->h_bout, ctx->d_bout, (M + 1) * sizeof(PointWords), hipMemcpyDeviceToHost, st));
  }
  if (ctx->profile >= 2) HIPCHK(hipEventRecord(ctx->ev[7], st));
  bc.M = M; bc.c = c; bc.nwin = nwin; bc.host_horner = host_horner; bc.h0 = h0; bc.h1 = std::chrono::steady_clock::now();
  return CG1_OK;
}

static int batched_chain_finish(Ctx* ctx, const BatchedChain& bc, cg1h::jac* results) {
  const size_t M = bc.M; const int c = bc.c; const uint32_t nwin = bc.nwin; const bool host_horner = bc.host_horner;
  const auto h0 = bc.h0, h1 = bc.h1;
  HIPCHK(hipSetDevice(ctx->device));
  { int wrc = wait_stream(ctx); if (wrc) return wrc; }
  HIPCHK(hipGetLastError());
  {
    const uint32_t* st_words = reinterpret_cast<const uint32_t*>(ctx->h_bout + M);
    ctx->last_entries = st_words[1]; ctx->last_chunks = st_words[2];
    if (st_words[0]) {
      snprintf(ctx->err, sizeof ctx->err, "a scalar is >= 2^255: scalar32 must be a canonical Fr element (< r)");
      return CG1_ERR_ENCODING;
    }
  }
  auto h2 = std::chrono::steady_clock::now();
  { int erc = read_phase_events(ctx, ctx->profile); if (erc) return erc; }
  ctx->last_c = c;
  if (host_horner) {
    auto one = [&](size_t j) {
      cg1h::jac a = cg1h::jac_identity();
      for (int w = (int)nwin - 1; w >= 0; --w) {
        for (int k = 0; k < c; ++k) a = cg1h::jac_dbl(a);
        a = cg1h::jac_add(a, jac_from_words(ctx->h_gout[j * nwin + (size_t)w]));
      }
      results[j] = a;
    };
    const size_t nth = std::min<size_t>(4, M);
    for (size_t t = 1; t < nth; ++t) ctx->helper[t - 1].run([&, t]() { for (size_t j = t; j < M; j += nth) one(j); });
    for (size_t j = 0; j < M; j += nth) one(j);
    for (size_t t = 1; t < nth; ++t) ctx->helper[t - 1].wait();
  } else {
    for (size_t j = 0; j < M; ++j) results[j] = jac_from_words(ctx->h_bout[j]);
  }
  auto h3 = std::chrono::steady_clock::now();
  ctx->host_ms[0] = std::chrono::duration<float, std::milli>(h1 - h0).count();
  ctx->host_ms[1] = std::chrono::duration<float, std::milli>(h2 - h1).count();
  ctx->host_ms[2] = 0;
  ctx->host_ms[3] = ctx->host_tail_ms = std::chrono::duration<float, std::milli>(h3 - h2).count();
  return CG1_OK;
}

static int msm_batched_small_end(Ctx* ctx, size_t M, std::vector<cg1h::jac>& results) {
  if (M == 1) { cg1h::jac r; int rc = msm_finish(ctx, r); ctx->last_acc_launches = 0; if (rc == CG1_OK) results[0] = r; return rc; }
  return msm_small_batched_finish(ctx, (uint32_t)M, results);
}
int msm_batched_device(Ctx* ctx, const void* d_points96, const void* d_scalars32, const uint32_t* h_offsets, size_t M,
                       int c, std::vector<cg1h::jac>& results, bool* async_small = nullptr, const uint32_t* d_offsets_ready = nullptr) {
  if (async_small) *async_small = false;
  results.assign(M, cg1h::jac_identity());
  if (M == 0) return CG1_OK;
  const size_t N = h_offsets[M];
  for (size_t j = 0; j < M; ++j) if (h_offsets[j] > h_offsets[j + 1]) { snprintf(ctx->err, sizeof ctx->err, "offsets not monotone"); return CG1_ERR_ARG; }
  if (h_offsets[0] != 0) { snprintf(ctx->err, sizeof ctx->err, "offsets[0] must be 0"); return CG1_ERR_ARG; }
  if (N == 0) return CG1_OK;
  if (N >= (1ull << 31) || M > 65535) { snprintf(ctx->err, sizeof ctx->err, "batch too large"); return CG1_ERR_ARG; }
  {
    size_t max_n = 0;
    for (size_t j = 0; j < M; ++j) max_n = std::max<size_t>(max_n, h_offsets[j + 1] - h_offsets[j]);
    const bool sglv = ctx->glv && 2 * max_n <= SM_MAX_N;
    const size_t max_nn = sglv ? 2 * max_n : max_n;
    const int cs = c > 0 ? c : pick_small_c(max_nn);
    const size_t groups = (size_t)M * (size_t)((sglv ? 127 : 255) / cs + 1) * ((max_nn + SM_SLICE - 1) / SM_SLICE);
    if (ctx->small_msm && M <= SM_MAX_MSMS && max_nn <= SM_MAX_N && groups <= SM_MAX_GROUPS && cs >= 4 && cs <= 9 && cs != 5) {
      HIPCHK(hipSetDevice(ctx->device));
      const uint32_t* d_offs = d_offsets_ready;
      if (!d_offs) {
        if ((M + 1) > ctx->cap_boffs) {
          if (ctx->d_boffs) (void)hipFree(ctx->d_boffs);
          ctx->d_boffs = nullptr; ctx->cap_boffs = 0;
          HIPCHK(hipMalloc(&ctx->d_boffs, (M + 1) * 4));
          ctx->cap_boffs = M + 1;
        }
        HIPCHK(hipMemcpyAsync(ctx->d_boffs, h_offsets, (M + 1) * 4, hipMemcpyHostToDevice, ctx->stream));
        d_offs = ctx->d_boffs;
      }
      int rc = msm_enqueue_small(ctx, PtSrc(d_points96), d_scalars32, N, cs, (uint32_t)M, d_offs, max_n, sglv);
      if (rc) return rc;
      if (async_small) { *async_small = true; return CG1_OK; }
      return msm_batched_small_end(ctx, M, results);
    }
  }
  const bool glv = ctx->glv != 0 && 2 * N < (1ull << 31);
  if (c <= 0) c = pick_window_batched((N + M - 1) / M, glv);
  if (c < 4 || c > 9) { snprintf(ctx->err, sizeof ctx->err, "batched window width %d out of range [4,9]", c); return CG1_ERR_ARG; }
  HIPCHK(hipSetDevice(ctx->device));
  if (!ctx->batched_split || M < (size_t)ctx->batched_split_min_m || h_offsets[M / 2] == 0 || h_offsets[M / 2] == N) {
    BatchedChain bc;
    int rc = batched_chain_enqueue(ctx, d_points96, d_scalars32, h_offsets, M, c, glv, nullptr, nullptr, bc);
    if (rc) return rc;
    return batched_chain_finish(ctx, bc, results.data());
  }
  { int crc = ensure_child(ctx); if (crc) return crc; }
  Ctx* ch = child_of(ctx);
  ch->profile = ctx->profile; ch->L0 = ctx->L0; ch->quad = ctx->quad; ch->horner_row = ctx->horner_row; ch->blocking_sync = ctx->blocking_sync;
  ch->batched_host_horner_max = ctx->batched_host_horner_max; ch->use_partition_sort = ctx->use_partition_sort;
  const size_t Mlo = M / 2, Mhi = M - Mlo;
  std::vector<uint32_t> offs_hi(Mhi + 1);
  for (size_t j = 0; j <= Mhi; ++j) offs_hi[j] = h_offsets[Mlo + j] - h_offsets[Mlo];
  BatchedChain lo, hi;
  int rc = batched_chain_enqueue(ctx, d_points96, d_scalars32, h_offsets, Mlo, c, glv, nullptr, ctx->ev_acc, lo);
  if (rc) return rc;
  rc = batched_chain_enqueue(ch, static_cast<const uint8_t*>(d_points96) + 96ull * h_offsets[Mlo], static_cast<const uint8_t*>(d_scalars32) + 32ull * h_offsets[Mlo],
                             offs_hi.data(), Mhi, c, glv, ctx->ev_acc, nullptr, hi);
  if (rc) { snprintf(ctx->err, sizeof ctx->err, "%s", ch->err); (void)batched_chain_finish(ctx, lo, results.data()); return rc; }
  rc = batched_chain_finish(ctx, lo, results.data());
  const float acc_lo = ctx->phase_ms[4], enq_lo = ctx->host_ms[0], wait_lo = ctx->host_ms[1];
  const uint32_t e_lo = ctx->last_entries, c_lo = ctx->last_chunks;
  int rc2 = batched_chain_finish(ch, hi, results.data() + Mlo);
  if (rc2 != CG1_OK) snprintf(ctx->err, sizeof ctx->err, "%s", ch->err);
  if (rc == CG1_OK) rc = rc2;
  ctx->phase_ms[4] = acc_lo + ch->phase_ms[4];
  ctx->last_entries = e_lo + ch->last_entries; ctx->last_chunks = c_lo + ch->last_chunks;
  ctx->host_ms[0] = enq_lo + ch->host_ms[0]; ctx->host_ms[1] = wait_lo + ch->host_ms[1];
  return rc;
}

}
```

curdleproofs_pie_amd/csrc/host_context.h:

```cpp
#pragma once

namespace cg1 {

#define HIPCHK(x) do { hipError_t e_ = (x); if (e_ != hipSuccess) { \
  snprintf(ctx->err, sizeof ctx->err, "%s failed: %s (%s:%d)", #x, hipGetErrorString(e_), __FILE__, __LINE__); return CG1_ERR_HIP; } } while (0)

struct Helper {
  std::thread th;
  std::mutex mu;
  std::condition_variable cv;
  std::function<void()> job;
  bool has = false, done = true, quit = false, armed = false;
  std::atomic<bool> posted{false};
  std::atomic<bool> stand_down{false};
  void start_locked() { if (!th.joinable()) th = std::thread([this]() { loop(); }); }
  void run(std::function<void()> f) {
    std::unique_lock<std::mutex> lk(mu);
    start_locked();
    job = std::move(f); has = true; done = false;
    posted.store(true, std::memory_order_release);
    cv.notify_all();
  }
  void arm() {
    std::unique_lock<std::mutex> lk(mu);
    start_locked();
    if (!has && done) { stand_down.store(false, std::memory_order_relaxed); armed = true; cv.notify_all(); }
  }
  void disarm() { stand_down.store(true, std::memory_order_release); }
  void wait() {
    std::unique_lock<std::mutex> lk(mu);
    cv.wait(lk, [this]() { return done; });
  }
  void loop() {
    std::unique_lock<std::mutex> lk(mu);
    for (;;) {
      cv.wait(lk, [this]() { return has || quit || armed; });
      if (quit) return;
      if (!has) {
        armed = false;
        lk.unlock();
        const auto until = std::chrono::steady_clock::now() + std::chrono::milliseconds(2);
        for (uint32_t k = 0; !posted.load(std::memory_order_acquire); ++k) {
          if (stand_down.load(std::memory_order_acquire)) break;
          if ((k & 0xffu) == 0xffu && std::chrono::steady_clock::now() > until) break;
          __builtin_ia32_pause();
        }
        lk.lock();
        if (!has) continue;
      }
      armed = false;
      std::function<void()> f = std::move(job);
      has = false;
      posted.store(false, std::memory_order_relaxed);
      lk.unlock();
      f();
      lk.lock();
      done = true;
      cv.notify_all();
    }
  }
  ~Helper() {
    { std::unique_lock<std::mutex> lk(mu); quit = true; cv.notify_all(); }
    if (th.joinable()) th.join();
  }
};

struct Ctx {
  int device = 0;
  Helper helper[3];
  hipStream_t stream = nullptr;
  std::atomic<hipStream_t> copy_stream{nullptr};
  std::once_flag copy_once;
  hipEvent_t copy_ev = nullptr;
  std::vector<uint32_t> cu_mask;
  hipStream_t side_stream = nullptr;
  hipEvent_t side_ev = nullptr;
  hipEvent_t sync_ev = nullptr;
  int blocking_sync = 0;
  char err[256] = {0};
  size_t cap_n = 0, cap_nb = 0, cap_chunks = 0, cap_entries = 0, cap_out = 0;
  PreparedPoint* d_pts = nullptr;
  uint8_t* d_flags = nullptr;
  uint32_t *d_hist = nullptr, *d_off = nullptr, *d_choff = nullptr, *d_sorted = nullptr;
  uint2 *d_blocktot = nullptr, *d_desc = nullptr;
  uint32_t *d_order = nullptr, *d_lenhist = nullptr;
  uint32_t* d_zblock = nullptr; size_t cap_zblock = 0;
  uint32_t* d_any_multi = nullptr;
  PointSum* d_partial = nullptr; size_t cap_partial = 0;
  uint16_t* d_digits = nullptr; uint32_t* d_part = nullptr; uint32_t* d_blockcnt = nullptr; uint32_t* d_ublocktot = nullptr;
  size_t cap_digits = 0, cap_part = 0, cap_blockcnt = 0;
  uint32_t *d_slice_base = nullptr, *d_slicehist = nullptr, *d_subbase = nullptr; uint8_t* d_bigflag = nullptr;
  size_t cap_bigflag = 0, cap_slices = 0;
  int big_bins = 1;
  int use_partition_sort = 1;
  int stage_sort = 1;
  int host_split = 1;
  int rowcol_quad = 1;
  int rowcol_lgq = 0;
  int rowcol_quad_max = 1 << 18;
  int tree_shift = 2;
  int tree_half = 1;
  int merlin_sync = 1;
  uint32_t merlin_clk[2] = {0, 0};
  int fe_timed = 0;
  int fe_rows = 1;
  int fe_prio = 0;
  int decompress_waves = 3;
  void* d_opening = nullptr; size_t cap_opening = 0;
  void* d_prover = nullptr; size_t cap_prover = 0;
  PreparedPoint* d_gen_tab = nullptr;
  int fixed_slice = 0;
  int fixed_waves = 0;
  int ipa_inv = 0;
  int merlin_last_kernel = 0;
  int merlin_rows = 1;
  void* d_merlin_rows = nullptr; size_t merlin_rows_cap = 0;
  int merlin_lanes = 64;
  uint32_t merlin_passes = 0;
  int sort_sub_bits = 0;
  int batch_mul_host_max = -1;
  int last_batch_mul_on_host = 0;
  int batch_mul_quad_max = 8192;
  int scan_one = 1;
  int fold_pass = 1;
  int auto_plan = 1;
  struct Pending {
    bool active = false;
    int c = 0, rank = 0, world = 1, nlw = 0, nbits = 0;
    WinPlan plan;
    uint32_t m = 1, lb2 = 0, hb2 = 0, nitems = 0;
    bool use2d = true;
    int profile = 0;
    bool zero_copy = false; uint32_t seq = 0;
    bool arm_helpers = false;
    size_t nout_words = 0;
    const PointWords* hout = nullptr;
    std::chrono::steady_clock::time_point h0, h1;
  } pend;
  int split = 0;
  size_t split_min_n = (size_t)1 << 17;
  cg1_ctx* child = nullptr;
  hipEvent_t ev_prep = nullptr, ev_acc = nullptr;
  bool pend_split = false;
  int last_acc_launches = 0;
  int small_row_tail = 1;
  int small_msm = 1;
  PointSum* d_small_partial = nullptr; size_t cap_small_partial = 0;
  uint32_t* d_small_ctr = nullptr;
  PreparedPoint* d_small_pts = nullptr; uint8_t* d_small_flags = nullptr; size_t cap_small_pts = 0;
  PointWords* h_small_out = nullptr; PointWords* h_small_out_dev = nullptr;
  int quad = 1;
  int reduce_2d = 1;
  uint32_t* d_heavy = nullptr; size_t cap_heavy = 0;
  uint8_t* d_combined = nullptr; size_t cap_combined = 0;
  uint32_t* d_boffs = nullptr; size_t cap_boffs = 0;
  PointSum* d_gsum = nullptr; size_t cap_gsum = 0;
  PointWords* d_bout = nullptr; PointWords* h_bout = nullptr; size_t cap_bout = 0;
  PointWords* d_gout = nullptr; PointWords* h_gout = nullptr; size_t cap_gout = 0;
  int glv = 0;
  int glv_max_n = 1 << 14;
  int lincomb_zero_copy = 1;
  int fold_quad = 1;
  int rowcol_row = 1;
  int tree_row = 1;
  int horner_row = 1;
  int batch_mul_row = 1;
  int batched_split = 0;
  int batched_split_min_m = 256;
  int batched_host_horner_max = 24;
  PointSum *d_sums = nullptr, *d_segrun = nullptr, *d_segtot = nullptr;
  PointWords* d_out = nullptr;
  PointWords* h_out = nullptr;
  PointWords* h_out_dev = nullptr;
  uint32_t* h_flag = nullptr;
  uint32_t* h_flag_dev = nullptr;
  uint32_t seq = 0;
  int zero_copy = 1;
  int arm_helpers = 1;
  int horner_threads = 4;
  void* d_stage_pts = nullptr; void* d_stage_sc = nullptr; size_t cap_stage_pts = 0, cap_stage_sc = 0;
  uint8_t* h_lin = nullptr; uint8_t* h_lin_dev = nullptr; size_t cap_h_lin = 0;
  hipEvent_t ev[CG1_NPHASE + 1];
  float phase_ms[CG1_NPHASE] = {0};
  float host_tail_ms = 0;
  float host_ms[4] = {0, 0, 0, 0};
  int profile = 1;
  uint32_t last_chunks = 0, last_entries = 0;
  hipEvent_t tm_ev[2] = {nullptr, nullptr};
  int last_c = 0, pend_c = 0;
  int chunk_rule = 1;
  uint32_t L0 = 8;
  uint32_t seg_m = 4;
};

static void free_bufs(Ctx* c) {
  auto F = [](auto*& p) { if (p) { (void)hipFree(p); p = nullptr; } };
  F(c->d_pts); F(c->d_flags); F(c->d_hist); F(c->d_off); F(c->d_choff); F(c->d_sorted); F(c->d_blocktot); F(c->d_desc);
  F(c->d_sums); F(c->d_segrun); F(c->d_segtot); F(c->d_out); F(c->d_order); F(c->d_zblock); F(c->d_partial);
  c->d_lenhist = c->d_heavy = c->d_any_multi = nullptr; c->d_combined = nullptr; c->cap_zblock = 0; c->cap_heavy = 0; c->cap_combined = 0;
  c->cap_partial = 0;
  F(c->d_digits); F(c->d_part); F(c->d_blockcnt); F(c->d_ublocktot); F(c->d_boffs); F(c->d_gsum); F(c->d_bout);
  F(c->d_slice_base); F(c->d_slicehist); F(c->d_subbase); F(c->d_bigflag); c->cap_bigflag = 0; c->cap_slices = 0;
  if (c->h_bout) { (void)hipHostFree(c->h_bout); c->h_bout = nullptr; }
  if (c->h_lin) { (void)hipHostFree(c->h_lin); c->h_lin = nullptr; c->h_lin_dev = nullptr; c->cap_h_lin = 0; }
  if (c->d_gout) { (void)hipFree(c->d_gout); c->d_gout = nullptr; }
  if (c->h_gout) { (void)hipHostFree(c->h_gout); c->h_gout = nullptr; }
  c->cap_gout = 0;
  c->cap_boffs = c->cap_gsum = c->cap_bout = 0;
  c->cap_digits = c->cap_part = c->cap_blockcnt = 0;
  if (c->h_out) { (void)hipHostFree(c->h_out); c->h_out = nullptr; }
  c->cap_n = c->cap_nb = c->cap_chunks = c->cap_entries = c->cap_out = 0;
}

static int ensure(Ctx* ctx, size_t n, size_t nb_total, size_t nlw, size_t nitems, uint32_t L, bool need_points = true) {
  size_t entries = n * nlw;
  size_t chunks = nb_total + entries / L + 1;
  if (need_points && n > ctx->cap_n) {
    if (ctx->d_pts) (void)hipFree(ctx->d_pts);
    if (ctx->d_flags) (void)hipFree(ctx->d_flags);
    HIPCHK(hipMalloc(&ctx->d_pts, n * sizeof(PreparedPoint)));
    HIPCHK(hipMalloc(&ctx->d_flags, n + 16));
    ctx->cap_n = n;
  }
  if (nb_total > ctx->cap_nb) {
    auto F = [](auto*& p) { if (p) { (void)hipFree(p); p = nullptr; } };
    F(ctx->d_hist); F(ctx->d_off); F(ctx->d_choff); F(ctx->d_blocktot); F(ctx->d_segrun); F(ctx->d_segtot);
    HIPCHK(hipMalloc(&ctx->d_hist, nb_total * 4));
    HIPCHK(hipMalloc(&ctx->d_off, (nb_total + 1) * 4));
    HIPCHK(hipMalloc(&ctx->d_choff, (nb_total + 1) * 4));
    HIPCHK(hipMalloc(&ctx->d_blocktot, (nb_total / SCAN_ITEMS + 2) * sizeof(uint2)));
    HIPCHK(hipMalloc(&ctx->d_segrun, nb_total * sizeof(PointSum)));
    HIPCHK(hipMalloc(&ctx->d_segtot, nb_total * sizeof(PointSum)));
    ctx->cap_nb = nb_total;
  }
  if (entries > ctx->cap_entries) {
    if (ctx->d_sorted) (void)hipFree(ctx->d_sorted);
    HIPCHK(hipMalloc(&ctx->d_sorted, (entries + 1) * 4));
    ctx->cap_entries = entries;
  }
  if (chunks > ctx->cap_chunks) {
    if (ctx->d_desc) (void)hipFree(ctx->d_desc);
    if (ctx->d_sums) (void)hipFree(ctx->d_sums);
    if (ctx->d_order) (void)hipFree(ctx->d_order);
    HIPCHK(hipMalloc(&ctx->d_order, chunks * 4));
    HIPCHK(hipMalloc(&ctx->d_desc, chunks * sizeof(uint2)));
    HIPCHK(hipMalloc(&ctx->d_sums, chunks * sizeof(PointSum)));
    ctx->cap_chunks = chunks;
  }
  {
    const size_t hcap = entries / ((size_t)L * (HEAVY_MIN_CHUNKS - 1)) + 2;
    const size_t z0 = 2 * LEN_BINS + 1, h0 = z0 + (nb_total + 3) / 4, words = h0 + 1 + hcap + 64;
    if (words > ctx->cap_zblock) {
      if (ctx->d_zblock) (void)hipFree(ctx->d_zblock);
      ctx->d_zblock = nullptr; ctx->cap_zblock = 0;
      HIPCHK(hipMalloc(&ctx->d_zblock, words * 4));
      ctx->cap_zblock = words;
    }
    ctx->d_lenhist = ctx->d_zblock;
    ctx->d_any_multi = ctx->d_zblock + 2 * LEN_BINS;
    ctx->d_combined = reinterpret_cast<uint8_t*>(ctx->d_zblock + z0);
    ctx->d_heavy = ctx->d_zblock + h0;
    ctx->cap_heavy = hcap;
    ctx->cap_combined = nb_total;
  }
  if (ctx->use_partition_sort && n <= PART_MAX_N) {
    const size_t nslices = (n + PART_TILE - 1) / PART_TILE;
    const size_t nbc = nlw * 128 * nslices + 1;
    if (entries > ctx->cap_digits) {
      if (ctx->d_digits) (void)hipFree(ctx->d_digits);
      HIPCHK(hipMalloc(&ctx->d_digits, entries * 2 + 16));
      ctx->cap_digits = entries;
    }
    if (entries > ctx->cap_part) {
      if (ctx->d_part) (void)hipFree(ctx->d_part);
      HIPCHK(hipMalloc(&ctx->d_part, (entries + 1) * 4));
      ctx->cap_part = entries;
    }
    if (nlw * 128 > ctx->cap_bigflag) {
      auto F = [](auto*& p) { if (p) { (void)hipFree(p); p = nullptr; } };
      F(ctx->d_bigflag); F(ctx->d_slice_base); F(ctx->d_subbase);
      HIPCHK(hipMalloc(&ctx->d_bigflag, nlw * 128 + 16));
      HIPCHK(hipMalloc(&ctx->d_slice_base, (nlw * 128 + 1) * 4));
      HIPCHK(hipMalloc(&ctx->d_subbase, nlw * 128 * 256 * 4));
      ctx->cap_bigflag = nlw * 128;
    }
    {
      const size_t max_slices = entries / SLICE + nlw * 128 + 1;
      if (max_slices > ctx->cap_slices) {
        if (ctx->d_slicehist) (void)hipFree(ctx->d_slicehist);
        HIPCHK(hipMalloc(&ctx->d_slicehist, max_slices * 256 * 4));
        ctx->cap_slices = max_slices;
      }
    }
    if (nbc > ctx->cap_blockcnt) {
      if (ctx->d_blockcnt) (void)hipFree(ctx->d_blockcnt);
      if (ctx->d_ublocktot) (void)hipFree(ctx->d_ublocktot);
      HIPCHK(hipMalloc(&ctx->d_blockcnt, nbc * 4));
      HIPCHK(hipMalloc(&ctx->d_ublocktot, (nbc / SCAN_ITEMS + 2) * 4));
      ctx->cap_blockcnt = nbc;
    }
  }
  size_t nout = nlw * nitems;
  if (nout * 64 > ctx->cap_partial) {
    if (ctx->d_partial) (void)hipFree(ctx->d_partial);
    HIPCHK(hipMalloc(&ctx->d_partial, nout * 64 * sizeof(PointSum)));
    ctx->cap_partial = nout * 64;
  }
  if (nout > ctx->cap_out) {
    if (ctx->d_out) (void)hipFree(ctx->d_out);
    if (ctx->h_out) (void)hipHostFree(ctx->h_out);
    HIPCHK(hipMalloc(&ctx->d_out, (nout + 1) * sizeof(PointWords)));
    HIPCHK(hipHostMalloc(&ctx->h_out, (nout + 1) * sizeof(PointWords), hipHostMallocMapped | hipHostMallocCoherent));
    HIPCHK(hipHostGetDevicePointer((void**)&ctx->h_out_dev, ctx->h_out, 0));
    ctx->cap_out = nout;
  }
  return CG1_OK;
}

static size_t zblock_clear_bytes(const Ctx* ctx) {
  size_t bytes = (size_t)((ctx->d_heavy + 1) - ctx->d_zblock) * 4;
  bytes = (bytes + 255) & ~(size_t)255;
  const size_t cap = ctx->cap_zblock * 4;
  return bytes < cap ? bytes : cap;
}

static int read_phase_events(Ctx* ctx, int profile) {
  for (int i = 0; i < CG1_NPHASE; ++i) ctx->phase_ms[i] = 0.f;
  if (profile >= 2) {
    for (int i = 0; i < CG1_NPHASE; ++i) HIPCHK(hipEventElapsedTime(&ctx->phase_ms[i], ctx->ev[i], ctx->ev[i + 1]));
  } else if (profile == 1) {
    HIPCHK(hipEventElapsedTime(&ctx->phase_ms[4], ctx->ev[4], ctx->ev[5]));
  }
  return CG1_OK;
}

static cg1h::fe fe_from_words12(const uint32_t w[12]) {
  cg1h::fe r;
  for (int i = 0; i < 6; ++i) r.l[i] = (uint64_t)w[2 * i] | ((uint64_t)w[2 * i + 1] << 32);
  return r;
}
static cg1h::jac jac_from_words(const PointWords& p) {
  if (p.inf) return cg1h::jac_identity();
  return cg1h::jac_from_xyzz(fe_from_words12(p.w[0]), fe_from_words12(p.w[1]), fe_from_words12(p.w[2]), fe_from_words12(p.w[3]));
}

}
```

curdleproofs_pie_amd/csrc/kernels_accumulate.h:

```cpp
#pragma once

__global__ void __launch_bounds__(256) k_accumulate(const uint2* __restrict__ desc, const uint32_t* __restrict__ total_chunks,
                                                    const uint32_t* __restrict__ order, const uint32_t* __restrict__ sorted,
                                                    const PreparedPoint* __restrict__ pts, PointSum* __restrict__ sums) {
  uint32_t g = blockIdx.x * 256 + threadIdx.x;
  if (g >= *total_chunks) return;
  const uint32_t t = order[g];
  const uint2 d = desc[t];
  const uint32_t* ent = sorted + d.x;
  if (d.y == 0u) { store_sum(sums + t, xyzz_identity()); return; }
  uint32_t e = ent[0];
  fp x, y; uint32_t flags;
  load_affine(pts + (e & 0x7fffffffu), x, y, flags);
  xyzz acc;
  uint32_t j = 1;
  if (e >> 31) y = fp_neg<3>(y);
  if (d.y >= 2u) {
    const uint32_t e1 = ent[1];
    fp x1, y1;
    load_affine(pts + (e1 & 0x7fffffffu), x1, y1, flags);
    if (e1 >> 31) y1 = fp_neg<3>(y1);
    e = ent[d.y > 2u ? 2 : 1];
    fp xn, yn;
    load_affine(pts + (e & 0x7fffffffu), xn, yn, flags);
    acc = xyzz_mmadd(x, y, x1, y1);
    x = xn; y = yn;
    j = 2;
  } else {
    acc = xyzz_from_affine(x, y);
  }
  for (; j < d.y; ++j) {
    const uint32_t en = ent[(j + 1 < d.y) ? j + 1 : j];
    fp xn, yn;
    load_affine(pts + (en & 0x7fffffffu), xn, yn, flags);
    if (e >> 31) y = fp_neg<3>(y);
    if (!xyzz_madd_fast(acc, x, y)) break;
    e = en; x = xn; y = yn;
  }
  for (; j < d.y; ++j) {
    acc = xyzz_madd(acc, x, y);
    if (j + 1 < d.y) {
      e = ent[j + 1];
      load_affine(pts + (e & 0x7fffffffu), x, y, flags);
      if (e >> 31) y = fp_neg<3>(y);
    }
  }
  store_sum(sums + t, acc);
}

__global__ void __launch_bounds__(256) k_heavy_combine(const uint32_t* __restrict__ heavy, uint32_t heavy_cap,
                                                       const uint32_t* __restrict__ choff, PointSum* __restrict__ sums,
                                                       uint8_t* __restrict__ combined) {
  __shared__ PointSum sh[4];
  uint32_t nheavy = heavy[0];
  if (nheavy > heavy_cap) nheavy = heavy_cap;
  for (uint32_t h = blockIdx.x; h < nheavy; h += gridDim.x) {
    const uint32_t b = heavy[1 + h];
    const uint32_t c0 = choff[b], c1 = choff[b + 1];
    xyzz acc = xyzz_identity();
    for (uint32_t k = c0 + threadIdx.x; k < c1; k += 256) acc = xyzz_add(acc, load_sum(sums + k));
    __syncthreads();
    for (int delta = 32; delta >= 1; delta >>= 1) {
      xyzz o = shfl_down_xyzz(acc, delta);
      if ((threadIdx.x & 63) < (uint32_t)delta) acc = xyzz_add(acc, o);
    }
    if ((threadIdx.x & 63) == 0) store_sum(&sh[threadIdx.x >> 6], acc);
    __syncthreads();
    if (threadIdx.x == 0) {
      for (int k = 1; k < 4; ++k) acc = xyzz_add(acc, load_sum(&sh[k]));
      store_sum(sums + c0, acc);
      combined[b] = 1;
    }
    __syncthreads();
  }
}

__global__ void __launch_bounds__(256) k_bucket_fold(const uint32_t* __restrict__ choff, PointSum* __restrict__ sums,
                                                     uint8_t* __restrict__ combined, uint32_t nb_total, const uint32_t* __restrict__ any_multi = nullptr) {
  if (any_multi && *any_multi == 0u) return;
  uint32_t b = blockIdx.x * 256 + threadIdx.x;
  if (b >= nb_total) return;
  const uint32_t c0 = choff[b], c1 = choff[b + 1];
  if (c1 - c0 < 2u || c1 - c0 >= HEAVY_MIN_CHUNKS) return;
  xyzz acc = load_sum(sums + c0);
  for (uint32_t k = c0 + 1; k < c1; ++k) acc = xyzz_add(acc, load_sum(sums + k));
  store_sum(sums + c0, acc);
  combined[b] = 1;
}
```

curdleproofs_pie_amd/csrc/kernels_sort.h:

```cpp
#pragma once

constexpr uint32_t PART_TILE = 4096;
constexpr uint32_t PART_MAX_N = 1u << 23;

__device__ __forceinline__ uint32_t digit_mag(uint32_t e, uint32_t& neg) {
  if (e == 0x8000u) { neg = 0; return 0x8000u; }
  int d = (int)(int16_t)(uint16_t)e;
  neg = d < 0;
  return (uint32_t)(d < 0 ? -d : d);
}

__device__ int g_wave_agg = 1;
__device__ __forceinline__ uint32_t lds_ranked_inc(uint32_t* ctr, uint32_t key, bool active) {
  if (!g_wave_agg) return active ? atomicAdd(&ctr[key], 1u) : 0u;
  const unsigned long long amask = __ballot(active);
  if (amask == 0ull) return 0u;
  const int leader = __ffsll((long long)amask) - 1;
  const uint32_t k0 = __shfl(key, leader, 64);
  if (__ballot(active && key != k0) == 0ull) {
    const uint32_t lane = threadIdx.x & 63u;
    uint32_t base = 0;
    if ((int)lane == leader) base = atomicAdd(&ctr[k0], (uint32_t)__popcll(amask));
    base = __shfl(base, leader, 64);
    return base + (uint32_t)__popcll(amask & ((1ull << lane) - 1ull));
  }
  return active ? atomicAdd(&ctr[key], 1u) : 0u;
}

__global__ void __launch_bounds__(256) k_digits(const uint32_t* __restrict__ scalars, const uint8_t* __restrict__ inf_flag,
                                                uint16_t* __restrict__ digits, uint32_t n, WinPlan pl, int rank, int world,
                                                uint32_t* __restrict__ bad_flag) {
  uint32_t i = blockIdx.x * 256 + threadIdx.x;
  if (i >= n) return;
  const bool inf = inf_flag[i] != 0;
  DigitIter it;
  load_scalar(scalars, i, it);
  if (it.s[7] >> 31) *bad_flag = 1u;
  if (pl.glv) {
    GlvParts g;
    glv_split(it.s, g);
    DigitIter a, b;
    load_half(g.k1, g.neg1, a);
    load_half(g.k2, g.neg2, b);
    const size_t nv = 2 * (size_t)n;
    WinWalk ww(rank, world);
    for (int w = 0; w < pl.nwin; ++w) {
      const int d1 = a.next(pl, w), d2 = b.next(pl, w);
      const int lw = ww.step(w);
      if (lw < 0) continue;
      digits[(size_t)lw * nv + i] = inf ? (uint16_t)0 : (uint16_t)(d1 & 0xFFFF);
      digits[(size_t)lw * nv + n + i] = inf ? (uint16_t)0 : (uint16_t)(d2 & 0xFFFF);
    }
    return;
  }
  WinWalk ww(rank, world);
  for (int w = 0; w < pl.nwin; ++w) {
    int d = it.next(pl, w);
    const int lw = ww.step(w);
    if (lw < 0) continue;
    digits[(size_t)lw * n + i] = inf ? (uint16_t)0 : (uint16_t)(d & 0xFFFF);
  }
}

__global__ void __launch_bounds__(256) k_part_count(const uint16_t* __restrict__ digits, uint32_t* __restrict__ block_counts,
                                                    uint32_t n, uint32_t nslices, uint32_t nbins, uint32_t sub_bits) {
  __shared__ uint32_t cnt[128];
  if (threadIdx.x < 128) cnt[threadIdx.x] = 0;
  __syncthreads();
  const uint32_t slice = blockIdx.x, lw = blockIdx.y;
  const uint16_t* dg = digits + (size_t)lw * n;
  for (uint32_t k = 0; k < PART_TILE / 256; ++k) {
    uint32_t i = slice * PART_TILE + k * 256 + threadIdx.x;
    uint32_t e = (i < n) ? (uint32_t)dg[i] : 0u;
    uint32_t neg, key = e ? ((digit_mag(e, neg) - 1u) >> sub_bits) : 0u;
    lds_ranked_inc(cnt, key, e != 0u);
  }
  __syncthreads();
  if (threadIdx.x < nbins) block_counts[((size_t)lw * nbins + threadIdx.x) * nslices + slice] = cnt[threadIdx.x];
}

__global__ void __launch_bounds__(256) k_part_scatter(const uint16_t* __restrict__ digits, const uint32_t* __restrict__ block_base,
                                                      uint32_t* __restrict__ part, uint32_t n, uint32_t nslices, uint32_t nbins,
                                                      uint32_t sub_bits, int use_stage) {
  __shared__ uint32_t cur[128];
  __shared__ uint32_t gbase[128];
  __shared__ uint32_t lbase[128];
  __shared__ uint32_t stage[PART_TILE];
  __shared__ uint32_t gpos[PART_TILE];
  const uint32_t slice = blockIdx.x, lw = blockIdx.y;
  uint32_t mycnt = 0;
  if (threadIdx.x < nbins) {
    const size_t idx = ((size_t)lw * nbins + threadIdx.x) * nslices + slice;
    gbase[threadIdx.x] = block_base[idx];
    mycnt = block_base[idx + 1] - block_base[idx];
    lbase[threadIdx.x] = mycnt;
  } else if (threadIdx.x < 128) {
    lbase[threadIdx.x] = 0;
  }
  __syncthreads();
  if (use_stage) {
    for (int d = 1; d < 128; d <<= 1) {
      uint32_t u = (threadIdx.x < 128 && (int)threadIdx.x >= d) ? lbase[threadIdx.x - d] : 0u;
      __syncthreads();
      if (threadIdx.x < 128) lbase[threadIdx.x] += u;
      __syncthreads();
    }
    if (threadIdx.x < 128) { lbase[threadIdx.x] -= mycnt; cur[threadIdx.x] = lbase[threadIdx.x]; }
  } else if (threadIdx.x < nbins) {
    cur[threadIdx.x] = gbase[threadIdx.x];
  }
  __syncthreads();
  const uint16_t* dg = digits + (size_t)lw * n;
  const uint32_t sub_mask = (1u << sub_bits) - 1u;
  for (uint32_t k = 0; k < PART_TILE / 256; ++k) {
    uint32_t i = slice * PART_TILE + k * 256 + threadIdx.x;
    uint32_t e = (i < n) ? (uint32_t)dg[i] : 0u;
    uint32_t neg = 0, b = e ? (digit_mag(e, neg) - 1u) : 0u;
    const uint32_t bin = b >> sub_bits;
    uint32_t pos = lds_ranked_inc(cur, bin, e != 0u);
    const uint32_t val = i | (neg << 23) | ((b & sub_mask) << 24);
    if (e) {
      if (use_stage) { stage[pos] = val; gpos[pos] = gbase[bin] + (pos - lbase[bin]); }
      else part[pos] = val;
    }
  }
  if (use_stage) {
    __syncthreads();
    const uint32_t total = lbase[nbins - 1] + (block_base[((size_t)lw * nbins + nbins - 1) * nslices + slice + 1] - gbase[nbins - 1]);
    for (uint32_t o = threadIdx.x; o < total; o += 256) part[gpos[o]] = stage[o];
  }
}
constexpr uint32_t BIN_STAGE = 12288;
__global__ void __launch_bounds__(256) k_bin_sort(const uint32_t* __restrict__ part, const uint32_t* __restrict__ block_base,
                                                  uint32_t* __restrict__ hist, uint32_t* __restrict__ sorted,
                                                  uint32_t nbins_total, uint32_t nslices, uint32_t sub_bits, int use_stage,
                                                  const uint8_t* __restrict__ bigflag) {
  __shared__ uint32_t cnt[256];
  __shared__ uint32_t cur[256];
  __shared__ uint32_t stage[BIN_STAGE];
  const uint32_t g = blockIdx.x;
  if (bigflag[g]) return;
  const uint32_t start = block_base[(size_t)g * nslices];
  const uint32_t end = block_base[(size_t)(g + 1) * nslices];
  cnt[threadIdx.x] = 0;
  __syncthreads();
  const uint32_t span = ((end - start + 255u) / 256u) * 256u;
  for (uint32_t o = threadIdx.x; o < span; o += 256) {
    const bool live = start + o < end;
    lds_ranked_inc(cnt, live ? (part[start + o] >> 24) : 0u, live);
  }
  __syncthreads();
  const uint32_t mine = cnt[threadIdx.x];
  cur[threadIdx.x] = mine;
  __syncthreads();
  for (int d = 1; d < 256; d <<= 1) {
    uint32_t u = ((int)threadIdx.x >= d) ? cur[threadIdx.x - d] : 0u;
    __syncthreads();
    cur[threadIdx.x] += u;
    __syncthreads();
  }
  const uint32_t excl = cur[threadIdx.x] - mine;
  __syncthreads();
  const bool staged = use_stage && (end - start) <= BIN_STAGE;
  cur[threadIdx.x] = (staged ? 0u : start) + excl;
  if (threadIdx.x < (1u << sub_bits)) hist[((size_t)g << sub_bits) + threadIdx.x] = mine;
  __syncthreads();
  for (uint32_t o = threadIdx.x; o < span; o += 256) {
    const bool live = start + o < end;
    const uint32_t v = live ? part[start + o] : 0u;
    const uint32_t pos = lds_ranked_inc(cur, v >> 24, live);
    const uint32_t val = (v & 0x7fffffu) | ((v >> 23 & 1u) << 31);
    if (live) { if (staged) stage[pos] = val; else sorted[pos] = val; }
  }
  if (staged) {
    __syncthreads();
    for (uint32_t o = threadIdx.x; start + o < end; o += 256) sorted[start + o] = stage[o];
  }
}

constexpr uint32_t SLICE = BIN_STAGE;

__global__ void __launch_bounds__(256) k_slice_plan(const uint32_t* __restrict__ block_base, uint32_t nbins_total, uint32_t nslices,
                                                    uint32_t* __restrict__ slice_base ,
                                                    uint8_t* __restrict__ bigflag, int enable) {
  __shared__ uint32_t part_sum[256];
  const uint32_t per = (nbins_total + 255u) / 256u, g0 = threadIdx.x * per;
  uint32_t mine = 0;
  for (uint32_t g = g0; g < g0 + per && g < nbins_total; ++g) {
    const uint32_t size = block_base[(size_t)(g + 1) * nslices] - block_base[(size_t)g * nslices];
    mine += (enable && size > BIN_STAGE) ? (size + SLICE - 1u) / SLICE : 0u;
  }
  part_sum[threadIdx.x] = mine;
  __syncthreads();
  for (int d = 1; d < 256; d <<= 1) {
    uint32_t u = ((int)threadIdx.x >= d) ? part_sum[threadIdx.x - d] : 0u;
    __syncthreads();
    part_sum[threadIdx.x] += u;
    __syncthreads();
  }
  uint32_t run = part_sum[threadIdx.x] - mine;
  for (uint32_t g = g0; g < g0 + per && g < nbins_total; ++g) {
    const uint32_t size = block_base[(size_t)(g + 1) * nslices] - block_base[(size_t)g * nslices];
    const uint32_t ns = (enable && size > BIN_STAGE) ? (size + SLICE - 1u) / SLICE : 0u;
    slice_base[g] = run;
    bigflag[g] = ns ? 1 : 0;
    run += ns;
  }
  if (threadIdx.x == 255) slice_base[nbins_total] = part_sum[255];
}

__device__ __forceinline__ bool slice_of_block(const uint32_t* __restrict__ slice_base, uint32_t nbins_total, uint32_t b,
                                               uint32_t& g, uint32_t& s) {
  if (b >= slice_base[nbins_total]) return false;
  uint32_t lo = 0, hi = nbins_total;
  while (hi - lo > 1) {
    const uint32_t mid = (lo + hi) >> 1;
    if (slice_base[mid] <= b) lo = mid; else hi = mid;
  }
  g = lo;
  s = b - slice_base[lo];
  return true;
}

__global__ void __launch_bounds__(256) k_slice_count(const uint32_t* __restrict__ part, const uint32_t* __restrict__ block_base,
                                                     uint32_t nbins_total, uint32_t nslices, const uint32_t* __restrict__ slice_base,
                                                     uint32_t* __restrict__ slicehist) {
  __shared__ uint32_t cnt[256];
  uint32_t g, s;
  if (!slice_of_block(slice_base, nbins_total, blockIdx.x, g, s)) return;
  const uint32_t start = block_base[(size_t)g * nslices], end = block_base[(size_t)(g + 1) * nslices];
  const uint32_t lo = start + s * SLICE, hi = (lo + SLICE < end) ? lo + SLICE : end;
  cnt[threadIdx.x] = 0;
  __syncthreads();
  const uint32_t span = ((hi - lo + 255u) / 256u) * 256u;
  for (uint32_t o = threadIdx.x; o < span; o += 256) {
    const bool live = lo + o < hi;
    lds_ranked_inc(cnt, live ? (part[lo + o] >> 24) : 0u, live);
  }
  __syncthreads();
  slicehist[(size_t)blockIdx.x * 256u + threadIdx.x] = cnt[threadIdx.x];
}

__global__ void __launch_bounds__(256) k_slice_prefix(const uint32_t* __restrict__ block_base, uint32_t nslices, uint32_t sub_bits,
                                                      const uint32_t* __restrict__ slice_base, const uint8_t* __restrict__ bigflag,
                                                      uint32_t* __restrict__ slicehist, uint32_t* __restrict__ subbase,
                                                      uint32_t* __restrict__ hist) {
  __shared__ uint32_t tot[256];
  const uint32_t g = blockIdx.x;
  if (!bigflag[g]) return;
  const uint32_t b0 = slice_base[g], b1 = slice_base[g + 1];
  uint32_t run = 0;
  for (uint32_t b = b0; b < b1; ++b) {
    const size_t idx = (size_t)b * 256u + threadIdx.x;
    const uint32_t v = slicehist[idx];
    slicehist[idx] = run;
    run += v;
  }
  tot[threadIdx.x] = run;
  __syncthreads();
  for (int d = 1; d < 256; d <<= 1) {
    uint32_t u = ((int)threadIdx.x >= d) ? tot[threadIdx.x - d] : 0u;
    __syncthreads();
    tot[threadIdx.x] += u;
    __syncthreads();
  }
  subbase[(size_t)g * 256u + threadIdx.x] = block_base[(size_t)g * nslices] + tot[threadIdx.x] - run;
  if (threadIdx.x < (1u << sub_bits)) hist[((size_t)g << sub_bits) + threadIdx.x] = run;
}

__global__ void __launch_bounds__(256) k_slice_scatter(const uint32_t* __restrict__ part, const uint32_t* __restrict__ block_base,
                                                       uint32_t nbins_total, uint32_t nslices, const uint32_t* __restrict__ slice_base,
                                                       const uint32_t* __restrict__ slicehist, const uint32_t* __restrict__ subbase,
                                                       uint32_t* __restrict__ sorted) {
  __shared__ uint32_t cnt[256];
  __shared__ uint32_t cur[256];
  __shared__ uint32_t gdst[256];
  __shared__ uint32_t stage[SLICE];
  uint32_t g, s;
  if (!slice_of_block(slice_base, nbins_total, blockIdx.x, g, s)) return;
  const uint32_t start = block_base[(size_t)g * nslices], end = block_base[(size_t)(g + 1) * nslices];
  const uint32_t lo = start + s * SLICE, hi = (lo + SLICE < end) ? lo + SLICE : end;
  cnt[threadIdx.x] = 0;
  __syncthreads();
  const uint32_t span = ((hi - lo + 255u) / 256u) * 256u;
  for (uint32_t o = threadIdx.x; o < span; o += 256) {
    const bool live = lo + o < hi;
    lds_ranked_inc(cnt, live ? (part[lo + o] >> 24) : 0u, live);
  }
  __syncthreads();
  const uint32_t mine = cnt[threadIdx.x];
  __syncthreads();
  for (int d = 1; d < 256; d <<= 1) {
    uint32_t u = ((int)threadIdx.x >= d) ? cnt[threadIdx.x - d] : 0u;
    __syncthreads();
    cnt[threadIdx.x] += u;
    __syncthreads();
  }
  const uint32_t lbase = cnt[threadIdx.x] - mine;
  __syncthreads();
  cnt[threadIdx.x] = lbase;
  cur[threadIdx.x] = lbase;
  gdst[threadIdx.x] = subbase[(size_t)g * 256u + threadIdx.x] + slicehist[(size_t)blockIdx.x * 256u + threadIdx.x];
  __syncthreads();
  for (uint32_t o = threadIdx.x; o < span; o += 256) {
    const bool live = lo + o < hi;
    const uint32_t v = live ? part[lo + o] : 0u;
    const uint32_t pos = lds_ranked_inc(cur, v >> 24, live);
    if (live) stage[pos] = v;
  }
  __syncthreads();
  for (uint32_t o = threadIdx.x; o < hi - lo; o += 256) {
    const uint32_t v = stage[o], k = v >> 24;
    sorted[gdst[k] + (o - cnt[k])] = (v & 0x7fffffu) | ((v >> 23 & 1u) << 31);
  }
}

__global__ void __launch_bounds__(256) k_uscan1(uint32_t* __restrict__ a, uint32_t* __restrict__ block_tot, uint32_t n) {
  __shared__ uint32_t sh[256];
  uint32_t base = blockIdx.x * SCAN_ITEMS + threadIdx.x * 4;
  uint32_t v[4], local = 0;
#pragma unroll
  for (int k = 0; k < 4; ++k) { v[k] = (base + k < n) ? a[base + k] : 0u; local += v[k]; }
  sh[threadIdx.x] = local;
  __syncthreads();
  for (int d = 1; d < 256; d <<= 1) {
    uint32_t u = ((int)threadIdx.x >= d) ? sh[threadIdx.x - d] : 0u;
    __syncthreads();
    sh[threadIdx.x] += u;
    __syncthreads();
  }
  uint32_t excl = sh[threadIdx.x] - local;
#pragma unroll
  for (int k = 0; k < 4; ++k) { if (base + k < n) a[base + k] = excl; excl += v[k]; }
  if (threadIdx.x == 255) block_tot[blockIdx.x] = sh[255];
}
__global__ void __launch_bounds__(256) k_uscan2(uint32_t* __restrict__ block_tot, uint32_t nblocks, uint32_t* __restrict__ a, uint32_t n) {
  __shared__ uint32_t sh[256];
  uint32_t carry = 0;
  for (uint32_t tile = 0; tile < nblocks; tile += 256) {
    uint32_t i = tile + threadIdx.x;
    uint32_t v = (i < nblocks) ? block_tot[i] : 0u;
    sh[threadIdx.x] = v;
    __syncthreads();
    for (int d = 1; d < 256; d <<= 1) {
      uint32_t u = ((int)threadIdx.x >= d) ? sh[threadIdx.x - d] : 0u;
      __syncthreads();
      sh[threadIdx.x] += u;
      __syncthreads();
    }
    if (i < nblocks) block_tot[i] = carry + sh[threadIdx.x] - v;
    uint32_t tot = sh[255];
    __syncthreads();
    carry += tot;
  }
  if (threadIdx.x == 0) a[n] = carry;
}
__global__ void __launch_bounds__(256) k_uscan3(const uint32_t* __restrict__ block_tot, uint32_t* __restrict__ a, uint32_t n) {
  uint32_t base = blockIdx.x * SCAN_ITEMS + threadIdx.x * 4;
  uint32_t p = block_tot[blockIdx.x];
#pragma unroll
  for (int k = 0; k < 4; ++k) if (base + k < n) a[base + k] += p;
}

constexpr uint32_t USCAN1_MAX = 1u << 15;
__global__ void __launch_bounds__(1024) k_uscan_one(uint32_t* __restrict__ a, uint32_t n) {
  __shared__ uint32_t sh[1024];
  const uint32_t per = (n + 1023u) / 1024u, lo = threadIdx.x * per, hi = (lo + per < n) ? lo + per : n;
  uint32_t local = 0;
  for (uint32_t i = lo; i < hi; ++i) local += a[i];
  sh[threadIdx.x] = local;
  __syncthreads();
  for (int d = 1; d < 1024; d <<= 1) {
    uint32_t u = ((int)threadIdx.x >= d) ? sh[threadIdx.x - d] : 0u;
    __syncthreads();
    sh[threadIdx.x] += u;
    __syncthreads();
  }
  uint32_t excl = sh[threadIdx.x] - local;
  for (uint32_t i = lo; i < hi; ++i) { const uint32_t v = a[i]; a[i] = excl; excl += v; }
  if (threadIdx.x == 1023) a[n] = sh[1023];
}

__global__ void __launch_bounds__(256) k_group_count(const uint16_t* __restrict__ digits, const uint32_t* __restrict__ offs,
                                                     uint32_t* __restrict__ hist, uint32_t N, uint32_t NB, uint32_t nwin, uint32_t split) {
  __shared__ uint32_t cnt[256];
  cnt[threadIdx.x] = 0;
  __syncthreads();
  const uint32_t j = blockIdx.x, w = blockIdx.y;
  const uint32_t o0 = offs[j], o1 = offs[j + 1];
  const uint32_t span = ((o1 - o0 + 255u) / 256u) * 256u;
  for (uint32_t half = 0; half < (split ? 2u : 1u); ++half) {
    const uint16_t* dg = digits + (size_t)w * N + (size_t)half * split;
    for (uint32_t o = threadIdx.x; o < span; o += 256) {
      const uint32_t e = (o0 + o < o1) ? (uint32_t)dg[o0 + o] : 0u;
      uint32_t neg;
      lds_ranked_inc(cnt, e ? digit_mag(e, neg) - 1u : 0u, e != 0u);
    }
  }
  __syncthreads();
  if (threadIdx.x < NB) hist[((size_t)j * nwin + w) * NB + threadIdx.x] = cnt[threadIdx.x];
}

__global__ void __launch_bounds__(256) k_group_scatter(const uint16_t* __restrict__ digits, const uint32_t* __restrict__ offs,
                                                       const uint32_t* __restrict__ off, uint32_t* __restrict__ sorted,
                                                       uint32_t N, uint32_t NB, uint32_t nwin, uint32_t split) {
  __shared__ uint32_t cur[256];
  const uint32_t j = blockIdx.x, w = blockIdx.y;
  if (threadIdx.x < NB) cur[threadIdx.x] = off[((size_t)j * nwin + w) * NB + threadIdx.x];
  __syncthreads();
  const uint32_t o0 = offs[j], o1 = offs[j + 1];
  const uint16_t* dg = digits + (size_t)w * N;
  const uint32_t span = ((o1 - o0 + 255u) / 256u) * 256u;
  for (uint32_t half = 0; half < (split ? 2u : 1u); ++half) {
    for (uint32_t o = threadIdx.x; o < span; o += 256) {
      const uint32_t i = half * split + o0 + o;
      const uint32_t e = (o0 + o < o1) ? (uint32_t)dg[i] : 0u;
      uint32_t neg = 0;
      const uint32_t b = e ? digit_mag(e, neg) - 1u : 0u;
      const uint32_t pos = lds_ranked_inc(cur, b, e != 0u);
      if (e) sorted[pos] = i | (neg << 31);
    }
  }
}

__global__ void __launch_bounds__(256) k_group_reduce(const PointSum* __restrict__ seg_run, const PointSum* __restrict__ seg_tot,
                                                      PointSum* __restrict__ group_sum, uint32_t ngroups, uint32_t J, uint32_t log2m) {
  uint32_t g = blockIdx.x * 256 + threadIdx.x;
  if (g >= ngroups) return;
  const PointSum* run = seg_run + (size_t)g * J;
  const PointSum* tot = seg_tot + (size_t)g * J;
  xyzz r = xyzz_identity(), t = xyzz_identity();
  for (uint32_t s = J - 1; s >= 1; --s) { r = xyzz_add(r, load_sum(run + s)); t = xyzz_add(t, r); }
  for (uint32_t k = 0; k < log2m; ++k) t = xyzz_dbl(t);
  for (uint32_t s = 0; s < J; ++s) t = xyzz_add(t, load_sum(tot + s));
  store_sum(group_sum + g, t);
}

__global__ void __launch_bounds__(64) k_msm_horner(const PointSum* __restrict__ group_sum, PointWords* __restrict__ out,
                                                   uint32_t M, uint32_t nwin, uint32_t c) {
  uint32_t j = blockIdx.x * 64 + threadIdx.x;
  if (j >= M) return;
  xyzz acc = xyzz_identity();
  for (int w = (int)nwin - 1; w >= 0; --w) {
    for (uint32_t k = 0; k < c; ++k) acc = xyzz_dbl(acc);
    acc = xyzz_add(acc, load_sum(group_sum + (size_t)j * nwin + w));
  }
  xyzz_words o;
  xyzz_export(acc, o);
  PointWords* dst = out + j;
  for (int cidx = 0; cidx < 4; ++cidx) for (int k = 0; k < 12; ++k) dst->w[cidx][k] = o.w[cidx][k];
  dst->inf = o.inf;
}

constexpr uint32_t MAX_CHUNKS_PER_BUCKET = 4096;
constexpr uint32_t HEAVY_MIN_CHUNKS = 17;
__device__ __forceinline__ uint32_t chunk_len(uint32_t cnt, uint32_t L0) {
  uint32_t s = (cnt + MAX_CHUNKS_PER_BUCKET - 1) / MAX_CHUNKS_PER_BUCKET;
  return s > L0 ? s : L0;
}
__device__ __forceinline__ uint32_t chunk_count(uint32_t cnt, uint32_t L0) {
  if (cnt == 0) return 0;
  uint32_t L = chunk_len(cnt, L0);
  return (cnt + L - 1) / L;
}

__global__ void __launch_bounds__(256) k_scan1(const uint32_t* __restrict__ hist, uint32_t* __restrict__ off, uint32_t* __restrict__ choff,
                                               uint2* __restrict__ block_tot, uint32_t nb_total, uint32_t L0) {
  __shared__ uint2 sh[256];
  uint32_t base = blockIdx.x * SCAN_ITEMS + threadIdx.x * 4;
  uint32_t cnt[4], ch[4];
  uint2 local = make_uint2(0, 0);
#pragma unroll
  for (int k = 0; k < 4; ++k) {
    cnt[k] = (base + k < nb_total) ? hist[base + k] : 0u;
    ch[k] = chunk_count(cnt[k], L0);
    local.x += cnt[k]; local.y += ch[k];
  }
  sh[threadIdx.x] = local;
  __syncthreads();
  for (int d = 1; d < 256; d <<= 1) {
    uint2 v = make_uint2(0, 0);
    if ((int)threadIdx.x >= d) v = sh[threadIdx.x - d];
    __syncthreads();
    sh[threadIdx.x].x += v.x; sh[threadIdx.x].y += v.y;
    __syncthreads();
  }
  uint2 excl = make_uint2(sh[threadIdx.x].x - local.x, sh[threadIdx.x].y - local.y);
#pragma unroll
  for (int k = 0; k < 4; ++k) {
    if (base + k < nb_total) { off[base + k] = excl.x; choff[base + k] = excl.y; }
    excl.x += cnt[k]; excl.y += ch[k];
  }
  if (threadIdx.x == 255) block_tot[blockIdx.x] = sh[255];
}
__global__ void __launch_bounds__(256) k_scan2(uint2* __restrict__ block_tot, uint32_t nblocks, uint32_t* __restrict__ off,
                                               uint32_t* __restrict__ choff, uint32_t nb_total) {
  __shared__ uint2 sh[256];
  uint2 carry = make_uint2(0, 0);
  for (uint32_t tile = 0; tile < nblocks; tile += 256) {
    uint32_t i = tile + threadIdx.x;
    uint2 v = (i < nblocks) ? block_tot[i] : make_uint2(0, 0);
    sh[threadIdx.x] = v;
    __syncthreads();
    for (int d = 1; d < 256; d <<= 1) {
      uint2 u = make_uint2(0, 0);
      if ((int)threadIdx.x >= d) u = sh[threadIdx.x - d];
      __syncthreads();
      sh[threadIdx.x].x += u.x; sh[threadIdx.x].y += u.y;
      __syncthreads();
    }
    if (i < nblocks) block_tot[i] = make_uint2(carry.x + sh[threadIdx.x].x - v.x, carry.y + sh[threadIdx.x].y - v.y);
    uint2 tot = sh[255];
    __syncthreads();
    carry.x += tot.x; carry.y += tot.y;
  }
  if (threadIdx.x == 0) { off[nb_total] = carry.x; choff[nb_total] = carry.y; }
}
__global__ void __launch_bounds__(256) k_scan3(const uint2* __restrict__ block_tot, uint32_t* __restrict__ off,
                                               uint32_t* __restrict__ choff, uint32_t nb_total) {
  uint32_t base = blockIdx.x * SCAN_ITEMS + threadIdx.x * 4;
  uint2 p = block_tot[blockIdx.x];
#pragma unroll
  for (int k = 0; k < 4; ++k) if (base + k < nb_total) { off[base + k] += p.x; choff[base + k] += p.y; }
}

constexpr uint32_t LEN_BINS = 256;
__device__ __forceinline__ uint32_t len_key(uint32_t len) { return len < LEN_BINS - 1 ? len : LEN_BINS - 1; }

constexpr uint32_t SCAN1_MAX = 1u << 13;
__global__ void __launch_bounds__(1024) k_scan_one(const uint32_t* __restrict__ hist, uint32_t* __restrict__ off, uint32_t* __restrict__ choff,
                                                    uint32_t nb_total, uint32_t L0) {
  __shared__ uint2 sh[1024];
  const uint32_t per = (nb_total + 1023u) / 1024u, lo = threadIdx.x * per, hi = (lo + per < nb_total) ? lo + per : nb_total;
  uint2 local = make_uint2(0, 0);
  for (uint32_t i = lo; i < hi; ++i) { const uint32_t c = hist[i]; local.x += c; local.y += chunk_count(c, L0); }
  sh[threadIdx.x] = local;
  __syncthreads();
  for (int d = 1; d < 1024; d <<= 1) {
    uint2 v = make_uint2(0, 0);
    if ((int)threadIdx.x >= d) v = sh[threadIdx.x - d];
    __syncthreads();
    sh[threadIdx.x].x += v.x; sh[threadIdx.x].y += v.y;
    __syncthreads();
  }
  uint2 excl = make_uint2(sh[threadIdx.x].x - local.x, sh[threadIdx.x].y - local.y);
  for (uint32_t i = lo; i < hi; ++i) {
    const uint32_t c = hist[i];
    off[i] = excl.x; choff[i] = excl.y;
    excl.x += c; excl.y += chunk_count(c, L0);
  }
  if (threadIdx.x == 1023) { off[nb_total] = sh[1023].x; choff[nb_total] = sh[1023].y; }
}

constexpr uint32_t CHUNK_DESC_BLOCKS = 320;
__global__ void __launch_bounds__(256) k_chunk_desc(const uint32_t* __restrict__ off, const uint32_t* __restrict__ choff,
                                                    uint2* __restrict__ desc, uint32_t* __restrict__ len_hist,
                                                    uint32_t* __restrict__ heavy ,
                                                    uint32_t heavy_cap, uint32_t nb_total, uint32_t L0, uint32_t* __restrict__ any_multi = nullptr) {
  __shared__ uint32_t sh[LEN_BINS];
  sh[threadIdx.x] = 0;
  __syncthreads();
#pragma unroll 1
  for (uint32_t b = blockIdx.x * 256 + threadIdx.x; b - threadIdx.x < nb_total; b += gridDim.x * 256) {
  if (b < nb_total) {
    uint32_t start = off[b], cnt = off[b + 1] - start;
    if (cnt) {
      uint32_t L = chunk_len(cnt, L0), nch = (cnt + L - 1) / L, o = choff[b];
      for (uint32_t k = 0; k < nch; ++k) {
        uint32_t s = k * L, len = (cnt - s < L) ? (cnt - s) : L;
        desc[o + k] = make_uint2(start + s, len);
      }
      if (nch > 1u) atomicAdd(&sh[len_key(L)], nch - 1u);
      atomicAdd(&sh[len_key(cnt - (nch - 1u) * L)], 1u);
      if (nch >= HEAVY_MIN_CHUNKS) {
        uint32_t slot = atomicAdd(&heavy[0], 1u);
        if (slot < heavy_cap) heavy[1 + slot] = b;
      } else if (nch >= 2u && any_multi) {
        *any_multi = 1u;
      }
    }
  }
  }
  __syncthreads();
  uint32_t v = sh[threadIdx.x];
  if (v) atomicAdd(&len_hist[threadIdx.x], v);
}

__global__ void __launch_bounds__(256) k_len_scan(const uint32_t* __restrict__ len_hist, uint32_t* __restrict__ len_cursor,
                                                  const uint32_t* __restrict__ total_entries, const uint32_t* __restrict__ total_chunks,
                                                  uint32_t* __restrict__ stats) {
  __shared__ uint32_t sh[LEN_BINS];
  if (threadIdx.x == 0) { stats[1] = *total_entries; stats[2] = *total_chunks; }
  uint32_t rev = LEN_BINS - 1 - threadIdx.x;
  uint32_t v = len_hist[rev];
  sh[threadIdx.x] = v;
  __syncthreads();
  for (int d = 1; d < 256; d <<= 1) {
    uint32_t u = ((int)threadIdx.x >= d) ? sh[threadIdx.x - d] : 0u;
    __syncthreads();
    sh[threadIdx.x] += u;
    __syncthreads();
  }
  len_cursor[rev] = sh[threadIdx.x] - v;
}

constexpr uint32_t ORDER_PER = 8;
__global__ void __launch_bounds__(256) k_order(const uint2* __restrict__ desc, const uint32_t* __restrict__ total_chunks,
                                               uint32_t* __restrict__ len_cursor, uint32_t* __restrict__ order) {
  __shared__ uint32_t cnt[LEN_BINS];
  __shared__ uint32_t base[LEN_BINS];
  cnt[threadIdx.x] = 0;
  __syncthreads();
  const uint32_t total = *total_chunks;
  uint32_t key[ORDER_PER], local[ORDER_PER];
#pragma unroll
  for (uint32_t rep = 0; rep < ORDER_PER; ++rep) {
    const uint32_t t = (blockIdx.x * ORDER_PER + rep) * 256 + threadIdx.x;
    const bool live = t < total;
    key[rep] = live ? len_key(desc[t].y) : 0u;
    local[rep] = 0;
    const unsigned long long amask = __ballot(live);
    if (amask) {
      const int leader = __ffsll((long long)amask) - 1;
      const uint32_t k0 = __shfl(key[rep], leader, 64);
      const unsigned long long same = __ballot(live && key[rep] == k0);
      const uint32_t lane = threadIdx.x & 63u;
      uint32_t b0 = 0;
      if ((int)lane == leader) b0 = atomicAdd(&cnt[k0], (uint32_t)__popcll(same));
      b0 = __shfl(b0, leader, 64);
      if (live) local[rep] = (key[rep] == k0) ? b0 + (uint32_t)__popcll(same & ((1ull << lane) - 1ull)) : atomicAdd(&cnt[key[rep]], 1u);
    }
  }
  __syncthreads();
  const uint32_t c = cnt[threadIdx.x];
  if (c) base[threadIdx.x] = atomicAdd(&len_cursor[threadIdx.x], c);
  __syncthreads();
#pragma unroll
  for (uint32_t rep = 0; rep < ORDER_PER; ++rep) {
    const uint32_t t = (blockIdx.x * ORDER_PER + rep) * 256 + threadIdx.x;
    if (t < total) order[base[key[rep]] + local[rep]] = t;
  }
}
```

Before: 373.2 million.

## Fuse MSM sort and fold kernels, drop memset, allow 8 Horner threads with late arming

Several MSM pipeline changes ship together. Digit extraction and partition counting are merged into one kernel. The zblock memset moves into the scan kernels. The bucket-fold pass moves into heavy_combine, and slice planning now runs only when big bins exist, with bin_sort setting the big flag itself. bin_sort keeps bin entries in registers instead of re-reading them, host Horner can use up to 8 threads, and a device flag lets large MSMs arm helper threads late. The aim is fewer launches and global passes and more host parallelism, at the cost of higher register pressure and more complex synchronization.

Result: no change. 379.3 million, median of 4 (+1.6%).

```diff
diff --git a/curdleproofs_pie_amd/csrc/capi_core_msm.h b/curdleproofs_pie_amd/csrc/capi_core_msm.h
--- a/curdleproofs_pie_amd/csrc/capi_core_msm.h
+++ b/curdleproofs_pie_amd/csrc/capi_core_msm.h
@@ -160,7 +160,7 @@
       hipEventCreateWithFlags(&ctx->sync_ev, hipEventDisableTiming | hipEventBlockingSync) != hipSuccess) { delete ctx; return nullptr; }
   for (int i = 0; i <= CG1_NPHASE; ++i) if (hipEventCreate(&ctx->ev[i]) != hipSuccess) { delete ctx; return nullptr; }
   if (hipHostMalloc((void**)&ctx->h_flag, 64, hipHostMallocMapped | hipHostMallocCoherent) != hipSuccess || hipHostGetDevicePointer((void**)&ctx->h_flag_dev, ctx->h_flag, 0) != hipSuccess) { delete ctx; return nullptr; }
-  *ctx->h_flag = 0;
+  ctx->h_flag[0] = ctx->h_flag[1] = 0;
   return ctx;
 }
 cg1_ctx* cg1_ctx_create(int device) { return cg1_ctx_create_cu_mask(device, nullptr, 0); }
@@ -297,7 +297,7 @@
   if (!strcmp(name, "big_bins")) { ctx->big_bins = value != 0; return CG1_OK; }
   if (!strcmp(name, "host_split")) { ctx->host_split = value != 0; return CG1_OK; }
   if (!strcmp(name, "arm_helpers")) { ctx->arm_helpers = value != 0; return CG1_OK; }
-  if (!strcmp(name, "horner_threads")) { if (value != 1 && value != 2 && value != 4) return CG1_ERR_ARG; ctx->horner_threads = value; return CG1_OK; }
+  if (!strcmp(name, "horner_threads")) { if (value != 1 && value != 2 && value != 4 && value != 8) return CG1_ERR_ARG; ctx->horner_threads = value; return CG1_OK; }
   if (!strcmp(name, "zero_copy")) { ctx->zero_copy = value != 0; return CG1_OK; }
   if (!strcmp(name, "auto_plan")) { ctx->auto_plan = value != 0; return CG1_OK; }
   if (!strcmp(name, "rowcol_quad")) { ctx->rowcol_quad = value != 0; return CG1_OK; }
diff --git a/curdleproofs_pie_amd/csrc/host_chains.h b/curdleproofs_pie_amd/csrc/host_chains.h
--- a/curdleproofs_pie_amd/csrc/host_chains.h
+++ b/curdleproofs_pie_amd/csrc/host_chains.h
@@ -122,6 +122,7 @@
   if (hooks.after_prepare) HIPCHK(hipEventRecord(hooks.after_prepare, st));
   if (profile >= 2) HIPCHK(hipEventRecord(ctx->ev[1], st));
   const uint32_t nblk = (uint32_t)((nb_total + SCAN_ITEMS - 1) / SCAN_ITEMS);
+  const uint32_t zwords = (uint32_t)(zblock_clear_bytes(ctx) / 4);
   if (ctx->use_partition_sort && n <= PART_MAX_N) {
     const uint32_t want_sub = ctx->sort_sub_bits ? (uint32_t)ctx->sort_sub_bits : (n <= ((size_t)1 << 16) ? 7u : 8u);
     uint32_t sub_bits = bb < want_sub ? bb : want_sub;
@@ -129,8 +130,8 @@
     const uint32_t nbins = 1u << (bb - sub_bits);
     const uint32_t nslices = (n32 + PART_TILE - 1) / PART_TILE;
     const uint32_t nbc = (uint32_t)nlw * nbins * nslices;
-    hipLaunchKernelGGL(k_digits, dim3((n_real32 + 255) / 256), dim3(256), 0, st, (const uint32_t*)d_scalars32, flags, ctx->d_digits, n_real32, plan, rank, world, bad_flag);
-    hipLaunchKernelGGL(k_part_count, dim3(nslices, nlw), dim3(256), 0, st, ctx->d_digits, ctx->d_blockcnt, n32, nslices, nbins, sub_bits);
+    hipLaunchKernelGGL(k_digits_count, dim3(nslices), dim3(DIG_THREADS), (size_t)nlw * nbins * 4, st, (const uint32_t*)d_scalars32, flags, ctx->d_digits, n_real32, plan, rank, world, bad_flag,
+                       ctx->d_blockcnt, nslices, nbins, sub_bits);
     const uint32_t ublk = (nbc + SCAN_ITEMS - 1) / SCAN_ITEMS;
     if (ctx->scan_one && nbc <= USCAN1_MAX) {
       hipLaunchKernelGGL(k_uscan_one, dim3(1), dim3(1024), 0, st, ctx->d_blockcnt, nbc);
@@ -143,9 +144,9 @@
     hipLaunchKernelGGL(k_part_scatter, dim3(nslices, nlw), dim3(256), 0, st, ctx->d_digits, ctx->d_blockcnt, ctx->d_part, n32, nslices, nbins, sub_bits, ctx->stage_sort);
     const uint32_t nbt = (uint32_t)nlw * nbins;
     const int big_bins = ctx->big_bins && n32 > 2u * BIN_STAGE;
-    hipLaunchKernelGGL(k_slice_plan, dim3(1), dim3(256), 0, st, ctx->d_blockcnt, nbt, nslices, ctx->d_slice_base, ctx->d_bigflag, big_bins);
-    hipLaunchKernelGGL(k_bin_sort, dim3(nbt), dim3(256), 0, st, ctx->d_part, ctx->d_blockcnt, ctx->d_hist, ctx->d_sorted, nbt, nslices, sub_bits, ctx->stage_sort, ctx->d_bigflag);
+    hipLaunchKernelGGL(k_bin_sort, dim3(nbt), dim3(256), 0, st, ctx->d_part, ctx->d_blockcnt, ctx->d_hist, ctx->d_sorted, nbt, nslices, sub_bits, ctx->stage_sort, ctx->d_bigflag, big_bins);
     if (big_bins) {
+      hipLaunchKernelGGL(k_slice_plan, dim3(1), dim3(256), 0, st, ctx->d_blockcnt, nbt, nslices, ctx->d_slice_base);
       const uint32_t max_slices = (uint32_t)(((size_t)n * (size_t)nlw) / SLICE + nbt + 1);
       hipLaunchKernelGGL(k_slice_count, dim3(max_slices), dim3(256), 0, st, ctx->d_part, ctx->d_blockcnt, nbt, nslices, ctx->d_slice_base, ctx->d_slicehist);
       hipLaunchKernelGGL(k_slice_prefix, dim3(nbt), dim3(256), 0, st, ctx->d_blockcnt, nslices, sub_bits, ctx->d_slice_base, ctx->d_bigflag, ctx->d_slicehist, ctx->d_subbase, ctx->d_hist);
@@ -153,9 +154,9 @@
     }
     if (profile >= 2) HIPCHK(hipEventRecord(ctx->ev[3], st));
     if (ctx->scan_one && nb_total <= SCAN1_MAX) {
-      hipLaunchKernelGGL(k_scan_one, dim3(1), dim3(1024), 0, st, ctx->d_hist, ctx->d_off, ctx->d_choff, (uint32_t)nb_total, L0);
+      hipLaunchKernelGGL(k_scan_one, dim3(1), dim3(1024), 0, st, ctx->d_hist, ctx->d_off, ctx->d_choff, (uint32_t)nb_total, L0, ctx->d_zblock, zwords);
     } else {
-      hipLaunchKernelGGL(k_scan1, dim3(nblk), dim3(256), 0, st, ctx->d_hist, ctx->d_off, ctx->d_choff, ctx->d_blocktot, (uint32_t)nb_total, L0);
+      hipLaunchKernelGGL(k_scan1, dim3(nblk), dim3(256), 0, st, ctx->d_hist, ctx->d_off, ctx->d_choff, ctx->d_blocktot, (uint32_t)nb_total, L0, ctx->d_zblock, zwords);
       hipLaunchKernelGGL(k_scan2, dim3(1), dim3(256), 0, st, ctx->d_blocktot, nblk, ctx->d_off, ctx->d_choff, (uint32_t)nb_total);
       hipLaunchKernelGGL(k_scan3, dim3(nblk), dim3(256), 0, st, ctx->d_blocktot, ctx->d_off, ctx->d_choff, (uint32_t)nb_total);
     }
@@ -163,13 +164,12 @@
     HIPCHK(hipMemsetAsync(ctx->d_hist, 0, nb_total * 4, st));
     hipLaunchKernelGGL(k_hist, dim3(gn), dim3(256), 0, st, (const uint32_t*)d_scalars32, flags, ctx->d_hist, n32, plan, rank, world, bad_flag);
     if (profile >= 2) HIPCHK(hipEventRecord(ctx->ev[2], st));
-    hipLaunchKernelGGL(k_scan1, dim3(nblk), dim3(256), 0, st, ctx->d_hist, ctx->d_off, ctx->d_choff, ctx->d_blocktot, (uint32_t)nb_total, L0);
+    hipLaunchKernelGGL(k_scan1, dim3(nblk), dim3(256), 0, st, ctx->d_hist, ctx->d_off, ctx->d_choff, ctx->d_blocktot, (uint32_t)nb_total, L0, ctx->d_zblock, zwords);
     hipLaunchKernelGGL(k_scan2, dim3(1), dim3(256), 0, st, ctx->d_blocktot, nblk, ctx->d_off, ctx->d_choff, (uint32_t)nb_total);
     hipLaunchKernelGGL(k_scan3, dim3(nblk), dim3(256), 0, st, ctx->d_blocktot, ctx->d_off, ctx->d_choff, (uint32_t)nb_total);
     if (profile >= 2) HIPCHK(hipEventRecord(ctx->ev[3], st));
     hipLaunchKernelGGL(k_scatter, dim3(gn), dim3(256), 0, st, (const uint32_t*)d_scalars32, flags, ctx->d_hist, ctx->d_off, ctx->d_sorted, n32, plan, rank, world);
   }
-  HIPCHK(hipMemsetAsync(ctx->d_zblock, 0, zblock_clear_bytes(ctx), st));
   hipLaunchKernelGGL(k_chunk_desc, dim3((uint32_t)std::min<size_t>(CHUNK_DESC_BLOCKS, (nb_total + 255) / 256)), dim3(256), 0, st, ctx->d_off, ctx->d_choff, ctx->d_desc, ctx->d_lenhist, ctx->d_heavy, (uint32_t)ctx->cap_heavy, (uint32_t)nb_total, L0, ctx->d_any_multi);
   const size_t max_chunks = nb_total + (n * (size_t)nlw) / L0 + 1;
   const uint32_t gchunks = (uint32_t)((max_chunks + 255) / 256);
@@ -180,14 +180,17 @@
   hipLaunchKernelGGL(k_accumulate, dim3(gchunks), dim3(256), 0, st, ctx->d_desc, ctx->d_choff + nb_total, ctx->d_order, ctx->d_sorted, pts, ctx->d_sums);
   if (profile >= 1) HIPCHK(hipEventRecord(ctx->ev[5], st));
   if (hooks.after_accumulate) HIPCHK(hipEventRecord(hooks.after_accumulate, st));
-  hipLaunchKernelGGL(k_heavy_combine, dim3(512), dim3(256), 0, st, ctx->d_heavy, (uint32_t)ctx->cap_heavy, ctx->d_choff, ctx->d_sums, ctx->d_combined);
   const bool small_quad = ctx->quad && ctx->rowcol_quad && nb_total <= (size_t)ctx->rowcol_quad_max;
   const bool rows_fold = small_quad && use2d && ctx->rowcol_row && ctx->tree_row && nb_total <= 8192;
+  const bool lane_fold = !rows_fold && !(small_quad && ctx->fold_quad) && ctx->fold_pass;
+  const bool zc_call = ctx->zero_copy != 0;
+  const bool arm_late = zc_call && ctx->arm_helpers && ctx->host_split && ctx->horner_threads > 1 && n > ((size_t)1 << 18);
+  hipLaunchKernelGGL(k_heavy_combine, dim3(lane_fold ? std::max<uint32_t>(512u, (uint32_t)((nb_total + 255) / 256)) : 512u), dim3(256), 0, st, ctx->d_heavy, (uint32_t)ctx->cap_heavy,
+                     ctx->d_choff, ctx->d_sums, ctx->d_combined, lane_fold ? (uint32_t)nb_total : 0u, (const uint32_t*)ctx->d_any_multi,
+                     arm_late ? ctx->h_flag_dev + 1 : (uint32_t*)nullptr, ctx->seq + 1u);
   if (rows_fold) {}
   else if (small_quad && ctx->fold_quad)
     hipLaunchKernelGGL(k_bucket_fold_quad, dim3((uint32_t)((nb_total * 4 + 255) / 256)), dim3(256), 0, st, ctx->d_choff, ctx->d_sums, ctx->d_combined, (uint32_t)nb_total, ctx->d_any_multi);
-  else if (ctx->fold_pass)
-    hipLaunchKernelGGL(k_bucket_fold, dim3((uint32_t)((nb_total + 255) / 256)), dim3(256), 0, st, ctx->d_choff, ctx->d_sums, ctx->d_combined, (uint32_t)nb_total, ctx->d_any_multi);
   bool tree_exports = false;
   if (use2d) {
     const uint32_t R = 1u << hb2, Cn = 1u << lb2;
@@ -230,7 +233,7 @@
     hipLaunchKernelGGL(k_bit_tree, dim3(nitems, nlw, S), dim3(256), 0, st, ctx->d_segrun, ctx->d_segtot, ctx->d_partial, J);
     hipLaunchKernelGGL(k_bit_tree_final, dim3((uint32_t)(nitems * nlw)), dim3(64), 0, st, ctx->d_partial, ctx->d_out, S);
   }
-  const bool zc = ctx->zero_copy != 0;
+  const bool zc = zc_call;
   if (zc && tree_exports) {
   } else if (zc) {
     ++ctx->seq;
@@ -247,6 +250,7 @@
   pd.active = true; pd.c = c; pd.plan = plan; pd.rank = rank; pd.world = world; pd.nlw = nlw; pd.nbits = nbits; pd.m = m; pd.lb2 = lb2; pd.hb2 = hb2;
   pd.nitems = nitems; pd.use2d = use2d; pd.profile = profile; pd.nout_words = nout_words; pd.h0 = h0; pd.h1 = h1;
   pd.arm_helpers = ctx->arm_helpers && ctx->host_split && ctx->horner_threads > 1 && n <= ((size_t)1 << 18);
+  pd.arm_late = arm_late;
   return CG1_OK;
 }
 
@@ -262,12 +266,14 @@
   const size_t nout_words = pd.nout_words;
   const auto h0 = pd.h0, h1 = pd.h1;
   HIPCHK(hipSetDevice(ctx->device));
-  struct StandDown { Ctx* c; bool on; ~StandDown() { if (on) for (int j = 0; j < 3; ++j) c->helper[j].disarm(); } } stand_down{ctx, false};
+  struct StandDown { Ctx* c; bool on; ~StandDown() { if (on) for (int j = 0; j < HORNER_HELPERS; ++j) c->helper[j].disarm(); } } stand_down{ctx, false};
+  bool armed = false;
   if (pd.zero_copy && !ctx->blocking_sync && pd.profile < 2) {
-    if (pd.arm_helpers) for (int j = 0; j < 3 && j + 1 < ctx->horner_threads; ++j) ctx->helper[j].arm();
-    stand_down.on = pd.arm_helpers;
+    auto arm = [&]() { for (int j = 0; j < HORNER_HELPERS && j + 1 < ctx->horner_threads; ++j) ctx->helper[j].arm(); armed = true; stand_down.on = true; };
+    if (pd.arm_helpers) arm();
     volatile uint32_t* flag = ctx->h_flag;
     for (uint32_t spins = 0; *flag != pd.seq; ++spins) {
+      if (pd.arm_late && !armed && flag[1] == pd.seq) arm();
       if ((spins & 0x3fffu) == 0x3fffu) {
         hipError_t q = hipStreamQuery(ctx->stream);
         if (q == hipSuccess) { if (*flag != pd.seq) { snprintf(ctx->err, sizeof ctx->err, "the stream drained without the export flag"); return CG1_ERR_HIP; } break; }
@@ -333,10 +339,10 @@
     return a;
   };
   cg1h::jac acc;
-  const int nth = (!ctx->host_split || e_top < 96) ? 1 : (ctx->horner_threads >= 4 && e_top >= 112 ? 4 : 2);
+  const int nth = (!ctx->host_split || e_top < 96) ? 1 : (ctx->horner_threads >= 4 && e_top >= 112 ? (ctx->horner_threads >= 8 && e_top >= 224 ? 8 : 4) : 2);
   if (nth > 1) {
-    cg1h::jac part[4];
-    int lo[5];
+    cg1h::jac part[HORNER_HELPERS + 1];
+    int lo[HORNER_HELPERS + 2];
     {
       constexpr long DBL = 7, ADD = 16;
       auto fill = [&](long C, int* cut) {
@@ -350,7 +356,7 @@
         return e > e_top;
       };
       long lo_c = DBL * (e_top + 1), hi_c = DBL * (e_top + 1) + ADD * (long)items.size();
-      int cut[5];
+      int cut[HORNER_HELPERS + 2];
       while (lo_c < hi_c) {
         const long mid = (lo_c + hi_c) / 2;
         if (fill(mid, cut)) hi_c = mid; else lo_c = mid + 1;
@@ -364,12 +370,12 @@
       part[j] = a;
     };
     for (int j = 0; j + 1 < nth; ++j) ctx->helper[j].run([&, j]() { run_part(j); });
-    if (pd.arm_helpers) for (int j = nth - 1 < 0 ? 0 : nth - 1; j < 3; ++j) ctx->helper[j].disarm();
+    if (armed) for (int j = nth - 1 < 0 ? 0 : nth - 1; j < HORNER_HELPERS; ++j) ctx->helper[j].disarm();
     run_part(nth - 1);
     acc = part[nth - 1];
     for (int j = 0; j + 1 < nth; ++j) { ctx->helper[j].wait(); acc = cg1h::jac_add(acc, part[j]); }
   } else {
-    if (pd.arm_helpers) for (int j = 0; j < 3; ++j) ctx->helper[j].disarm();
+    if (armed) for (int j = 0; j < HORNER_HELPERS; ++j) ctx->helper[j].disarm();
     acc = horner(0, e_top);
   }
   result = acc;
@@ -440,6 +446,7 @@
   pd.active = true; pd.c = c; pd.plan = plan; pd.rank = 0; pd.world = 1; pd.nlw = (int)nwin; pd.nbits = 0; pd.m = 1; pd.lb2 = lb2; pd.hb2 = hb2;
   pd.nitems = nitems; pd.use2d = true; pd.profile = 0; pd.nout_words = (size_t)M * nwin * nitems; pd.h0 = h0; pd.h1 = h1;
   pd.arm_helpers = ctx->arm_helpers && ctx->host_split && ctx->horner_threads > 1 && M == 1;
+  pd.arm_late = false;
   return CG1_OK;
 }
 
@@ -658,12 +665,12 @@
   hipLaunchKernelGGL(k_group_count, dim3((uint32_t)M, nwin), dim3(256), 0, st, ctx->d_digits, ctx->d_boffs, ctx->d_hist, Nv32, NB, nwin, split);
   if (ctx->profile >= 2) HIPCHK(hipEventRecord(ctx->ev[2], st));
   const uint32_t nblk = (uint32_t)((nb_total + SCAN_ITEMS - 1) / SCAN_ITEMS);
-  hipLaunchKernelGGL(k_scan1, dim3(nblk), dim3(256), 0, st, ctx->d_hist, ctx->d_off, ctx->d_choff, ctx->d_blocktot, (uint32_t)nb_total, L0);
+  hipLaunchKernelGGL(k_scan1, dim3(nblk), dim3(256), 0, st, ctx->d_hist, ctx->d_off, ctx->d_choff, ctx->d_blocktot, (uint32_t)nb_total, L0, ctx->d_zblock,
+                     (uint32_t)(zblock_clear_bytes(ctx) / 4));
   hipLaunchKernelGGL(k_scan2, dim3(1), dim3(256), 0, st, ctx->d_blocktot, nblk, ctx->d_off, ctx->d_choff, (uint32_t)nb_total);
   hipLaunchKernelGGL(k_scan3, dim3(nblk), dim3(256), 0, st, ctx->d_blocktot, ctx->d_off, ctx->d_choff, (uint32_t)nb_total);
   hipLaunchKernelGGL(k_group_scatter, dim3((uint32_t)M, nwin), dim3(256), 0, st, ctx->d_digits, ctx->d_boffs, ctx->d_off, ctx->d_sorted, Nv32, NB, nwin, split);
   if (ctx->profile >= 2) HIPCHK(hipEventRecord(ctx->ev[3], st));
-  HIPCHK(hipMemsetAsync(ctx->d_zblock, 0, zblock_clear_bytes(ctx), st));
   hipLaunchKernelGGL(k_chunk_desc, dim3((uint32_t)std::min<size_t>(CHUNK_DESC_BLOCKS, (nb_total + 255) / 256)), dim3(256), 0, st, ctx->d_off, ctx->d_choff, ctx->d_desc, ctx->d_lenhist, ctx->d_heavy, (uint32_t)ctx->cap_heavy, (uint32_t)nb_total, L0, ctx->d_any_multi);
   const size_t max_chunks = nb_total + (Nv * (size_t)nwin) / L0 + 1;
   const uint32_t gchunks = (uint32_t)((max_chunks + 255) / 256);
@@ -675,7 +682,8 @@
   if (ctx->profile >= 1) HIPCHK(hipEventRecord(ctx->ev[5], st));
   if (record_after_accumulate) HIPCHK(hipEventRecord(record_after_accumulate, st));
   const uint32_t nseg_total = (uint32_t)(nb_total / m);
-  hipLaunchKernelGGL(k_heavy_combine, dim3(512), dim3(256), 0, st, ctx->d_heavy, (uint32_t)ctx->cap_heavy, ctx->d_choff, ctx->d_sums, ctx->d_combined);
+  hipLaunchKernelGGL(k_heavy_combine, dim3(512), dim3(256), 0, st, ctx->d_heavy, (uint32_t)ctx->cap_heavy, ctx->d_choff, ctx->d_sums, ctx->d_combined, 0u, (const uint32_t*)nullptr,
+                     (uint32_t*)nullptr, 0u);
   hipLaunchKernelGGL(k_seg_reduce, dim3((nseg_total + 255) / 256), dim3(256), 0, st, ctx->d_choff, ctx->d_sums, ctx->d_combined, ctx->d_segrun, ctx->d_segtot, nseg_total, m);
   hipLaunchKernelGGL(k_group_reduce, dim3((uint32_t)((G + 255) / 256)), dim3(256), 0, st, ctx->d_segrun, ctx->d_segtot, ctx->d_gsum, (uint32_t)G, J, log2m);
   if (ctx->profile >= 2) HIPCHK(hipEventRecord(ctx->ev[6], st));
diff --git a/curdleproofs_pie_amd/csrc/host_context.h b/curdleproofs_pie_amd/csrc/host_context.h
--- a/curdleproofs_pie_amd/csrc/host_context.h
+++ b/curdleproofs_pie_amd/csrc/host_context.h
@@ -65,9 +65,10 @@
   }
 };
 
+constexpr int HORNER_HELPERS = 7;
 struct Ctx {
   int device = 0;
-  Helper helper[3];
+  Helper helper[HORNER_HELPERS];
   hipStream_t stream = nullptr;
   std::atomic<hipStream_t> copy_stream{nullptr};
   std::once_flag copy_once;
@@ -133,6 +134,7 @@
     int profile = 0;
     bool zero_copy = false; uint32_t seq = 0;
     bool arm_helpers = false;
+    bool arm_late = false;
     size_t nout_words = 0;
     const PointWords* hout = nullptr;
     std::chrono::steady_clock::time_point h0, h1;
diff --git a/curdleproofs_pie_amd/csrc/kernels_accumulate.h b/curdleproofs_pie_amd/csrc/kernels_accumulate.h
--- a/curdleproofs_pie_amd/csrc/kernels_accumulate.h
+++ b/curdleproofs_pie_amd/csrc/kernels_accumulate.h
@@ -48,10 +48,14 @@
   store_sum(sums + t, acc);
 }
 
+__device__ __forceinline__ void bucket_fold_lane(const uint32_t* __restrict__ choff, PointSum* __restrict__ sums, uint8_t* __restrict__ combined,
+                                                 uint32_t nb_total, const uint32_t* __restrict__ any_multi);
 __global__ void __launch_bounds__(256) k_heavy_combine(const uint32_t* __restrict__ heavy, uint32_t heavy_cap,
                                                        const uint32_t* __restrict__ choff, PointSum* __restrict__ sums,
-                                                       uint8_t* __restrict__ combined) {
+                                                       uint8_t* __restrict__ combined, uint32_t fold_nb, const uint32_t* __restrict__ any_multi,
+                                                       uint32_t* __restrict__ begun_host, uint32_t seq) {
   __shared__ PointSum sh[4];
+  if (begun_host && blockIdx.x == 0 && threadIdx.x == 0) __hip_atomic_store(begun_host, seq, __ATOMIC_RELAXED, __HIP_MEMORY_SCOPE_SYSTEM);
   uint32_t nheavy = heavy[0];
   if (nheavy > heavy_cap) nheavy = heavy_cap;
   for (uint32_t h = blockIdx.x; h < nheavy; h += gridDim.x) {
@@ -73,10 +77,11 @@
     }
     __syncthreads();
   }
+  if (fold_nb) bucket_fold_lane(choff, sums, combined, fold_nb, any_multi);
 }
 
-__global__ void __launch_bounds__(256) k_bucket_fold(const uint32_t* __restrict__ choff, PointSum* __restrict__ sums,
-                                                     uint8_t* __restrict__ combined, uint32_t nb_total, const uint32_t* __restrict__ any_multi = nullptr) {
+__device__ __forceinline__ void bucket_fold_lane(const uint32_t* __restrict__ choff, PointSum* __restrict__ sums, uint8_t* __restrict__ combined,
+                                                 uint32_t nb_total, const uint32_t* __restrict__ any_multi) {
   if (any_multi && *any_multi == 0u) return;
   uint32_t b = blockIdx.x * 256 + threadIdx.x;
   if (b >= nb_total) return;
diff --git a/curdleproofs_pie_amd/csrc/kernels_sort.h b/curdleproofs_pie_amd/csrc/kernels_sort.h
--- a/curdleproofs_pie_amd/csrc/kernels_sort.h
+++ b/curdleproofs_pie_amd/csrc/kernels_sort.h
@@ -62,21 +62,58 @@
   }
 }
 
-__global__ void __launch_bounds__(256) k_part_count(const uint16_t* __restrict__ digits, uint32_t* __restrict__ block_counts,
-                                                    uint32_t n, uint32_t nslices, uint32_t nbins, uint32_t sub_bits) {
-  __shared__ uint32_t cnt[128];
-  if (threadIdx.x < 128) cnt[threadIdx.x] = 0;
-  __syncthreads();
-  const uint32_t slice = blockIdx.x, lw = blockIdx.y;
-  const uint16_t* dg = digits + (size_t)lw * n;
-  for (uint32_t k = 0; k < PART_TILE / 256; ++k) {
-    uint32_t i = slice * PART_TILE + k * 256 + threadIdx.x;
-    uint32_t e = (i < n) ? (uint32_t)dg[i] : 0u;
-    uint32_t neg, key = e ? ((digit_mag(e, neg) - 1u) >> sub_bits) : 0u;
-    lds_ranked_inc(cnt, key, e != 0u);
-  }
-  __syncthreads();
-  if (threadIdx.x < nbins) block_counts[((size_t)lw * nbins + threadIdx.x) * nslices + slice] = cnt[threadIdx.x];
+constexpr uint32_t DIG_THREADS = 1024, DIG_PER = PART_TILE / DIG_THREADS;
+__global__ void __launch_bounds__(DIG_THREADS) k_digits_count(const uint32_t* __restrict__ scalars, const uint8_t* __restrict__ inf_flag,
+                                                              uint16_t* __restrict__ digits, uint32_t n, WinPlan pl, int rank, int world,
+                                                              uint32_t* __restrict__ bad_flag, uint32_t* __restrict__ block_counts,
+                                                              uint32_t nslices, uint32_t nbins, uint32_t sub_bits) {
+  extern __shared__ uint32_t dc_cnt[];
+  const uint32_t ncnt = (uint32_t)win_count(pl.nwin, rank, world) * nbins;
+  for (uint32_t x = threadIdx.x; x < ncnt; x += DIG_THREADS) dc_cnt[x] = 0;
+  const uint32_t nv = pl.glv ? 2u * n : n, tile = blockIdx.x;
+  auto fetch = [&](uint32_t k, uint4& lo, uint4& hi, uint32_t& inf) {
+    const uint32_t j = tile * PART_TILE + k * DIG_THREADS + threadIdx.x;
+    const uint32_t i = j < nv ? (j >= n ? j - n : j) : 0u;
+    const uint4* q = reinterpret_cast<const uint4*>(scalars + 8ull * i);
+    lo = q[0]; hi = q[1]; inf = inf_flag[i];
+  };
+  uint4 lo, hi; uint32_t inf;
+  fetch(0, lo, hi, inf);
+  __syncthreads();
+#pragma unroll 1
+  for (uint32_t k = 0; k < DIG_PER; ++k) {
+    const uint32_t j = tile * PART_TILE + k * DIG_THREADS + threadIdx.x;
+    const bool live = j < nv;
+    DigitIter it;
+    it.s[0] = lo.x; it.s[1] = lo.y; it.s[2] = lo.z; it.s[3] = lo.w;
+    it.s[4] = hi.x; it.s[5] = hi.y; it.s[6] = hi.z; it.s[7] = hi.w;
+    it.carry = 0; it.flip = 0;
+    const bool dead = !live || inf != 0u;
+    if (k + 1 < DIG_PER) fetch(k + 1, lo, hi, inf);
+    if (live && (it.s[7] >> 31)) *bad_flag = 1u;
+    if (pl.glv) {
+      GlvParts g;
+      glv_split(it.s, g);
+      const bool second = j >= n;
+      uint32_t mag[4];
+#pragma unroll
+      for (int q = 0; q < 4; ++q) mag[q] = second ? g.k2[q] : g.k1[q];
+      load_half(mag, second ? g.neg2 : g.neg1, it);
+    }
+    WinWalk ww(rank, world);
+    for (int w = 0; w < pl.nwin; ++w) {
+      const int d = it.next(pl, w);
+      const int lw = ww.step(w);
+      if (lw < 0) continue;
+      const uint32_t e = dead ? 0u : (uint32_t)(d & 0xFFFF);
+      if (live) digits[(size_t)lw * nv + j] = (uint16_t)e;
+      uint32_t neg;
+      const uint32_t key = e ? ((digit_mag(e, neg) - 1u) >> sub_bits) : 0u;
+      lds_ranked_inc(dc_cnt + (uint32_t)lw * nbins, key, e != 0u);
+    }
+  }
+  __syncthreads();
+  for (uint32_t x = threadIdx.x; x < ncnt; x += DIG_THREADS) block_counts[(size_t)x * nslices + tile] = dc_cnt[x];
 }
 
 __global__ void __launch_bounds__(256) k_part_scatter(const uint16_t* __restrict__ digits, const uint32_t* __restrict__ block_base,
@@ -88,6 +125,13 @@
   __shared__ uint32_t stage[PART_TILE];
   __shared__ uint32_t gpos[PART_TILE];
   const uint32_t slice = blockIdx.x, lw = blockIdx.y;
+  const uint16_t* dg = digits + (size_t)lw * n;
+  uint32_t e[PART_TILE / 256];
+#pragma unroll
+  for (uint32_t k = 0; k < PART_TILE / 256; ++k) {
+    const uint32_t i = slice * PART_TILE + k * 256 + threadIdx.x;
+    e[k] = (i < n) ? (uint32_t)dg[i] : 0u;
+  }
   uint32_t mycnt = 0;
   if (threadIdx.x < nbins) {
     const size_t idx = ((size_t)lw * nbins + threadIdx.x) * nslices + slice;
@@ -110,16 +154,15 @@
     cur[threadIdx.x] = gbase[threadIdx.x];
   }
   __syncthreads();
-  const uint16_t* dg = digits + (size_t)lw * n;
   const uint32_t sub_mask = (1u << sub_bits) - 1u;
+#pragma unroll
   for (uint32_t k = 0; k < PART_TILE / 256; ++k) {
-    uint32_t i = slice * PART_TILE + k * 256 + threadIdx.x;
-    uint32_t e = (i < n) ? (uint32_t)dg[i] : 0u;
-    uint32_t neg = 0, b = e ? (digit_mag(e, neg) - 1u) : 0u;
+    const uint32_t i = slice * PART_TILE + k * 256 + threadIdx.x;
+    uint32_t neg = 0, b = e[k] ? (digit_mag(e[k], neg) - 1u) : 0u;
     const uint32_t bin = b >> sub_bits;
-    uint32_t pos = lds_ranked_inc(cur, bin, e != 0u);
+    uint32_t pos = lds_ranked_inc(cur, bin, e[k] != 0u);
     const uint32_t val = i | (neg << 23) | ((b & sub_mask) << 24);
-    if (e) {
+    if (e[k]) {
       if (use_stage) { stage[pos] = val; gpos[pos] = gbase[bin] + (pos - lbase[bin]); }
       else part[pos] = val;
     }
@@ -131,23 +174,64 @@
   }
 }
 constexpr uint32_t BIN_STAGE = 12288;
+constexpr uint32_t BIN_REGS = BIN_STAGE / 256;
+constexpr uint32_t BIN_BATCH = 8;
 __global__ void __launch_bounds__(256) k_bin_sort(const uint32_t* __restrict__ part, const uint32_t* __restrict__ block_base,
                                                   uint32_t* __restrict__ hist, uint32_t* __restrict__ sorted,
                                                   uint32_t nbins_total, uint32_t nslices, uint32_t sub_bits, int use_stage,
-                                                  const uint8_t* __restrict__ bigflag) {
+                                                  uint8_t* __restrict__ bigflag, int big_enable) {
   __shared__ uint32_t cnt[256];
   __shared__ uint32_t cur[256];
   __shared__ uint32_t stage[BIN_STAGE];
   const uint32_t g = blockIdx.x;
-  if (bigflag[g]) return;
   const uint32_t start = block_base[(size_t)g * nslices];
   const uint32_t end = block_base[(size_t)(g + 1) * nslices];
+  const uint32_t size = end - start;
+  const bool big = big_enable && size > BIN_STAGE;
+  if (threadIdx.x == 0) bigflag[g] = big ? 1 : 0;
+  if (big) return;
+  const bool in_regs = size <= BIN_STAGE;
+  const uint32_t* src = part + start;
+  uint32_t v[BIN_REGS], slot[BIN_REGS];
   cnt[threadIdx.x] = 0;
-  __syncthreads();
-  const uint32_t span = ((end - start + 255u) / 256u) * 256u;
-  for (uint32_t o = threadIdx.x; o < span; o += 256) {
-    const bool live = start + o < end;
-    lds_ranked_inc(cnt, live ? (part[start + o] >> 24) : 0u, live);
+  if (in_regs) {
+#pragma unroll
+    for (uint32_t b0 = 0; b0 < BIN_REGS; b0 += BIN_BATCH) {
+      if (b0 * 256u < size) {
+#pragma unroll
+        for (uint32_t k = b0; k < b0 + BIN_BATCH; ++k) {
+          const uint32_t o = k * 256u + threadIdx.x;
+          v[k] = src[o < size ? o : 0u];
+        }
+      }
+    }
+  }
+  __syncthreads();
+  if (in_regs) {
+#pragma unroll
+    for (uint32_t b0 = 0; b0 < BIN_REGS; b0 += BIN_BATCH) {
+      if (b0 * 256u < size) {
+#pragma unroll
+        for (uint32_t k = b0; k < b0 + BIN_BATCH; ++k) {
+          const bool live = k * 256u + threadIdx.x < size;
+          slot[k] = lds_ranked_inc(cnt, live ? (v[k] >> 24) : 0u, live);
+        }
+      }
+    }
+  } else {
+    for (uint32_t base = 0; base < size; base += BIN_BATCH * 256u) {
+      uint32_t w[BIN_BATCH];
+#pragma unroll
+      for (uint32_t k = 0; k < BIN_BATCH; ++k) {
+        const uint32_t o = base + k * 256u + threadIdx.x;
+        w[k] = src[o < size ? o : 0u];
+      }
+#pragma unroll
+      for (uint32_t k = 0; k < BIN_BATCH; ++k) {
+        const bool live = base + k * 256u + threadIdx.x < size;
+        lds_ranked_inc(cnt, live ? (w[k] >> 24) : 0u, live);
+      }
+    }
   }
   __syncthreads();
   const uint32_t mine = cnt[threadIdx.x];
@@ -161,34 +245,56 @@
   }
   const uint32_t excl = cur[threadIdx.x] - mine;
   __syncthreads();
-  const bool staged = use_stage && (end - start) <= BIN_STAGE;
+  const bool staged = use_stage && in_regs;
   cur[threadIdx.x] = (staged ? 0u : start) + excl;
   if (threadIdx.x < (1u << sub_bits)) hist[((size_t)g << sub_bits) + threadIdx.x] = mine;
   __syncthreads();
-  for (uint32_t o = threadIdx.x; o < span; o += 256) {
-    const bool live = start + o < end;
-    const uint32_t v = live ? part[start + o] : 0u;
-    const uint32_t pos = lds_ranked_inc(cur, v >> 24, live);
-    const uint32_t val = (v & 0x7fffffu) | ((v >> 23 & 1u) << 31);
-    if (live) { if (staged) stage[pos] = val; else sorted[pos] = val; }
+  if (in_regs) {
+#pragma unroll
+    for (uint32_t b0 = 0; b0 < BIN_REGS; b0 += BIN_BATCH) {
+      if (b0 * 256u < size) {
+#pragma unroll
+        for (uint32_t k = b0; k < b0 + BIN_BATCH; ++k) {
+          if (k * 256u + threadIdx.x < size) {
+            const uint32_t pos = cur[v[k] >> 24] + slot[k];
+            const uint32_t val = (v[k] & 0x7fffffu) | ((v[k] >> 23 & 1u) << 31);
+            if (staged) stage[pos] = val; else sorted[pos] = val;
+          }
+        }
+      }
+    }
+  } else {
+    for (uint32_t base = 0; base < size; base += BIN_BATCH * 256u) {
+      uint32_t w[BIN_BATCH];
+#pragma unroll
+      for (uint32_t k = 0; k < BIN_BATCH; ++k) {
+        const uint32_t o = base + k * 256u + threadIdx.x;
+        w[k] = src[o < size ? o : 0u];
+      }
+#pragma unroll
+      for (uint32_t k = 0; k < BIN_BATCH; ++k) {
+        const bool live = base + k * 256u + threadIdx.x < size;
+        const uint32_t pos = lds_ranked_inc(cur, live ? (w[k] >> 24) : 0u, live);
+        if (live) sorted[pos] = (w[k] & 0x7fffffu) | ((w[k] >> 23 & 1u) << 31);
+      }
+    }
   }
   if (staged) {
     __syncthreads();
-    for (uint32_t o = threadIdx.x; start + o < end; o += 256) sorted[start + o] = stage[o];
+    for (uint32_t o = threadIdx.x; o < size; o += 256) sorted[start + o] = stage[o];
   }
 }
 
 constexpr uint32_t SLICE = BIN_STAGE;
 
 __global__ void __launch_bounds__(256) k_slice_plan(const uint32_t* __restrict__ block_base, uint32_t nbins_total, uint32_t nslices,
-                                                    uint32_t* __restrict__ slice_base ,
-                                                    uint8_t* __restrict__ bigflag, int enable) {
+                                                    uint32_t* __restrict__ slice_base ) {
   __shared__ uint32_t part_sum[256];
   const uint32_t per = (nbins_total + 255u) / 256u, g0 = threadIdx.x * per;
   uint32_t mine = 0;
   for (uint32_t g = g0; g < g0 + per && g < nbins_total; ++g) {
     const uint32_t size = block_base[(size_t)(g + 1) * nslices] - block_base[(size_t)g * nslices];
-    mine += (enable && size > BIN_STAGE) ? (size + SLICE - 1u) / SLICE : 0u;
+    mine += size > BIN_STAGE ? (size + SLICE - 1u) / SLICE : 0u;
   }
   part_sum[threadIdx.x] = mine;
   __syncthreads();
@@ -201,9 +307,8 @@
   uint32_t run = part_sum[threadIdx.x] - mine;
   for (uint32_t g = g0; g < g0 + per && g < nbins_total; ++g) {
     const uint32_t size = block_base[(size_t)(g + 1) * nslices] - block_base[(size_t)g * nslices];
-    const uint32_t ns = (enable && size > BIN_STAGE) ? (size + SLICE - 1u) / SLICE : 0u;
+    const uint32_t ns = size > BIN_STAGE ? (size + SLICE - 1u) / SLICE : 0u;
     slice_base[g] = run;
-    bigflag[g] = ns ? 1 : 0;
     run += ns;
   }
   if (threadIdx.x == 255) slice_base[nbins_total] = part_sum[255];
@@ -465,8 +570,10 @@
 }
 
 __global__ void __launch_bounds__(256) k_scan1(const uint32_t* __restrict__ hist, uint32_t* __restrict__ off, uint32_t* __restrict__ choff,
-                                               uint2* __restrict__ block_tot, uint32_t nb_total, uint32_t L0) {
+                                               uint2* __restrict__ block_tot, uint32_t nb_total, uint32_t L0,
+                                               uint32_t* __restrict__ zblock, uint32_t zwords) {
   __shared__ uint2 sh[256];
+  for (uint32_t x = blockIdx.x * 256 + threadIdx.x; x < zwords; x += gridDim.x * 256) zblock[x] = 0u;
   uint32_t base = blockIdx.x * SCAN_ITEMS + threadIdx.x * 4;
   uint32_t cnt[4], ch[4];
   uint2 local = make_uint2(0, 0);
@@ -529,8 +636,9 @@
 
 constexpr uint32_t SCAN1_MAX = 1u << 13;
 __global__ void __launch_bounds__(1024) k_scan_one(const uint32_t* __restrict__ hist, uint32_t* __restrict__ off, uint32_t* __restrict__ choff,
-                                                    uint32_t nb_total, uint32_t L0) {
+                                                    uint32_t nb_total, uint32_t L0, uint32_t* __restrict__ zblock, uint32_t zwords) {
   __shared__ uint2 sh[1024];
+  for (uint32_t x = threadIdx.x; x < zwords; x += 1024) zblock[x] = 0u;
   const uint32_t per = (nb_total + 1023u) / 1024u, lo = threadIdx.x * per, hi = (lo + per < nb_total) ? lo + per : nb_total;
   uint2 local = make_uint2(0, 0);
   for (uint32_t i = lo; i < hi; ++i) { const uint32_t c = hist[i]; local.x += c; local.y += chunk_count(c, L0); }
```
